# LinXueyuanStdio/LaTeX_OCR

Hardware: AMD Instinct MI355X
Metric: formula-images/sec training step (batch 64, 128x512) (higher is better)
Workload: dtype bf16

## Files before the change

latex_ocr_amd/csrc/conv_igemm.hip:

```cpp
#include "gemm.h"
#include "api_util.h"
#include "decoder_kernels.h"
#include "lxo_debug.h"
#include <stdlib.h>

namespace {

__device__ unsigned lxo_zero_line[8] = {0, 0, 0, 0, 0, 0, 0, 0};

constexpr int CBM = 256, CBN = 128, CBK = 64, CTH = 512;
constexpr int A_STAGE = CBM * CBK * 2, B_STAGE = CBN * CBK * 2, STAGE = A_STAGE + B_STAGE;

typedef __attribute__((address_space(1))) const void* gptr_t;
typedef __attribute__((address_space(3))) void* lptr_t;
LXO_DEV void glds16(const void* g, void* l) {
    __builtin_amdgcn_global_load_lds((gptr_t)(uintptr_t)g, (lptr_t)(uintptr_t)l, 16, 0, 0);
}

}

HIP_DYNAMIC_SHARED(char, lxo_conv_lds)

namespace {

constexpr int HTH = 4, HTW = 64, HPW = HTW + 2, HPH = HTH + 2, HPROWS = HPH * HPW;
constexpr int HPSLOTS = 7 * CTH;
constexpr int HPATCH = HPSLOTS * 16, HB_STAGE = CBN * CBK * 2;

#ifdef LXO_DIAG
#define LXO_DIAG_BIT(b) (p.diag & (b))
#else
#define LXO_DIAG_BIT(b) false
#endif
#define LXO_VMCNT(n) __builtin_amdgcn_s_waitcnt(0x0F70 | ((n) & 15) | (((n) >> 4) << 14))
#define LXO_LDS_BARRIER() do { __builtin_amdgcn_s_waitcnt(0xC07F); __builtin_amdgcn_s_barrier(); } while (0)

template <typename OT, int NJ>
__global__ __launch_bounds__(512) void conv_halo_kernel(GemmNT p, int tiles_n, int tiles_x, int tiles_y) {
    constexpr int BN = 64 * NJ, HBS = BN * CBK * 2;
    const int tid = threadIdx.x, lane = tid & 63, wave = tid >> 6;
    const int wm = wave >> 1, wn = wave & 1;
    const int nblk = gridDim.x, bid = blockIdx.x;
    const int q = nblk >> 3, r8 = nblk & 7, xcd = bid & 7, slot = bid >> 3;
    const int tile = (xcd < r8 ? xcd * (q + 1) : r8 * (q + 1) + (xcd - r8) * q) + slot;
    const int mt = tile / tiles_n, nt = tile - mt * tiles_n;
    const int tx_i = mt % tiles_x, ty_i = (mt / tiles_x) % tiles_y, b = mt / (tiles_x * tiles_y);
    const int oy0 = ty_i * HTH, ox0 = tx_i * HTW, n0 = nt * BN;
    const bf16_t* __restrict__ A = reinterpret_cast<const bf16_t*>(p.A);
    const bf16_t* __restrict__ Bp = reinterpret_cast<const bf16_t*>(p.Bp);
    const char* zline = reinterpret_cast<const char*>(lxo_zero_line);
    char* patch0 = lxo_conv_lds;
    char* bst0 = lxo_conv_lds + 2 * HPATCH;

    const int sch = tid & 7;
    long long a_off[7];
    int a_gch[7];
#pragma unroll
    for (int j = 0; j < 7; ++j) {
        const int prow = (tid >> 3) + 64 * j;
        const int py = prow / HPW, px = prow - py * HPW;
        const int iy = oy0 + py - p.pad, ix = ox0 + px - p.pad;
        const bool ok = prow < HPROWS && iy >= 0 && iy < p.H && ix >= 0 && ix < p.W;
        a_off[j] = ok ? (((long long)b * p.H + iy) * p.W + ix) * p.Cin : -1;
        a_gch[j] = (sch ^ ((prow >> 1) & 7)) << 3;
    }
    const int srow = tid >> 3;
    const bf16_t* b_ptr[NJ]; bool b_ok[NJ];
#pragma unroll
    for (int j = 0; j < NJ; ++j) {
        const int n = n0 + srow + 64 * j;
        b_ok[j] = n < p.N;
        b_ptr[j] = Bp + (long long)(b_ok[j] ? n : 0) * p.ldb + ((sch ^ ((srow >> 1) & 7)) << 3);
    }
    auto issue_patch = [&](int c, int buf) {
        char* dst = patch0 + buf * HPATCH;
#pragma unroll
        for (int j = 0; j < 7; ++j) {
            const void* src = a_off[j] >= 0 ? (const void*)(A + a_off[j] + c * CBK + a_gch[j]) : (const void*)zline;
            glds16(src, dst + (wave * 64 + 512 * j) * 16);
        }
    };
    auto issue_b = [&](int t, int stage) {
        const int c = t / 9, tap = t - 9 * c;
        const int k0 = tap * p.Cin + c * CBK;
        char* dst = bst0 + stage * HBS;
#pragma unroll
        for (int j = 0; j < NJ; ++j) {
            const void* src = b_ok[j] ? (const void*)(b_ptr[j] + k0) : (const void*)zline;
            glds16(src, dst + (wave * 64 + 512 * j) * 16);
        }
    };

    f32x16 acc[2][NJ];
#pragma unroll
    for (int i = 0; i < 2; ++i)
#pragma unroll
        for (int j = 0; j < NJ; ++j)
#pragma unroll
            for (int e = 0; e < 16; ++e) acc[i][j][e] = 0.f;

    int a_prow[2];
#pragma unroll
    for (int i = 0; i < 2; ++i) {
        const int rr = wm * 64 + i * 32 + (lane & 31);
        a_prow[i] = (rr >> 6) * HPW + (rr & 63);
    }
    int b_row[NJ];
#pragma unroll
    for (int j = 0; j < NJ; ++j) b_row[j] = wn * 32 * NJ + j * 32 + (lane & 31);

    const int nchunk = p.Cin / CBK, nk = nchunk * 9;
    issue_patch(0, 0);
    issue_b(0, 0);
    if (nk > 1) issue_b(1, 1);
    for (int t = 0; t < nk; ++t) {
        const int tm = t % 9;
        const bool patch_after = (tm == 5 || tm == 6) && (t / 9 + 1 < nchunk);
        const int nafter = ((t + 1 < nk) ? NJ : 0) + (patch_after ? 7 : 0);
        if (nafter == NJ + 7) LXO_VMCNT(NJ + 7);
        else if (nafter == 7) LXO_VMCNT(7);
        else if (nafter == NJ) LXO_VMCNT(NJ);
        else LXO_VMCNT(0);
        __builtin_amdgcn_s_barrier();
        if (t + 2 < nk) issue_b(t + 2, (t + 2) % 3);
        if (tm == 4 && t / 9 + 1 < nchunk) issue_patch(t / 9 + 1, (t / 9 + 1) & 1);
        const int c = t / 9, tap = t - 9 * c;
        const int kh = tap / 3, kw = tap - 3 * kh;
        const char* ps = patch0 + (c & 1) * HPATCH;
        const char* bs = bst0 + (t % 3) * HBS;
        const int shift = kh * HPW + kw;
#pragma unroll
        for (int ks = 0; ks < 4; ++ks) {
            const int kc = ks * 2 + (lane >> 5);
            u32x4 af[2], bfr[NJ];
#pragma unroll
            for (int i = 0; i < 2; ++i) {
                const int prow = a_prow[i] + shift;
                af[i] = *reinterpret_cast<const u32x4*>(ps + prow * 128 + ((kc ^ ((prow >> 1) & 7)) << 4));
            }
#pragma unroll
            for (int j = 0; j < NJ; ++j)
                bfr[j] = *reinterpret_cast<const u32x4*>(bs + b_row[j] * 128 + ((kc ^ ((b_row[j] >> 1) & 7)) << 4));
#pragma unroll
            for (int i = 0; i < 2; ++i)
#pragma unroll
                for (int j = 0; j < NJ; ++j)
                    acc[i][j] = __builtin_amdgcn_mfma_f32_32x32x16_bf16(__builtin_bit_cast(bf16x8_t, af[i]), __builtin_bit_cast(bf16x8_t, bfr[j]),
                                                                        acc[i][j], 0, 0, 0);
        }
    }

    OT* __restrict__ C = reinterpret_cast<OT*>(p.C);
    const bool plain = !p.out_pre && !p.addend && !p.relu_ref && !p.colsum && !p.accumulate && p.ldc == p.N && (p.N & 7) == 0;
    if (plain) {
        LXO_LDS_BARRIER();
        bf16_t* ot = reinterpret_cast<bf16_t*>(lxo_conv_lds);
        constexpr int OP = BN + 8;
#pragma unroll
        for (int j = 0; j < NJ; ++j) {
            const int nl = wn * 32 * NJ + j * 32 + (lane & 31);
            const int n = n0 + nl;
            const float bias = (p.bias && n < p.N) ? p.bias[n] : 0.f;
#pragma unroll
            for (int i = 0; i < 2; ++i)
#pragma unroll
                for (int e = 0; e < 16; ++e) {
                    const int ml = wm * 64 + i * 32 + (e & 3) + 8 * (e >> 2) + 4 * (lane >> 5);
                    float v = p.alpha * acc[i][j][e] + bias;
                    if (p.act == 1) v = fmaxf(v, 0.f);
                    else if (p.act == 2) v = tanhf(v);
                    ot[ml * OP + nl] = f2bf(v);
                }
        }
        LXO_LDS_BARRIER();
#pragma unroll
        for (int it = 0; it < 4 * NJ; ++it) {
            const int idx = tid + 512 * it, row = idx / (BN / 8), c8 = (idx % (BN / 8)) * 8;
            const int oy = oy0 + (row >> 6), ox = ox0 + (row & 63), n = n0 + c8;
            if (oy < p.Ho && ox < p.Wo && n < p.N)
                *reinterpret_cast<u32x4*>(C + (((long long)b * p.Ho + oy) * p.Wo + ox) * p.ldc + n) = *reinterpret_cast<const u32x4*>(ot + row * OP + c8);
        }
        return;
    }
    OT* __restrict__ Cpre = reinterpret_cast<OT*>(p.out_pre);
    const bf16_t* __restrict__ ref = reinterpret_cast<const bf16_t*>(p.relu_ref);
#pragma unroll
    for (int j = 0; j < NJ; ++j) {
        const int n = n0 + wn * 32 * NJ + j * 32 + (lane & 31);
        const bool n_ok = n < p.N;
        const float bias = (p.bias && n_ok) ? p.bias[n] : 0.f;
        float csum = 0.f;
#pragma unroll
        for (int i = 0; i < 2; ++i) {
#pragma unroll
            for (int e = 0; e < 16; ++e) {
                const int ml = wm * 64 + i * 32 + (e & 3) + 8 * (e >> 2) + 4 * (lane >> 5);
                const int oy = oy0 + (ml >> 6), ox = ox0 + (ml & 63);
                if (!(n_ok && oy < p.Ho && ox < p.Wo)) continue;
                const long long m = ((long long)b * p.Ho + oy) * p.Wo + ox;
                float v = p.alpha * acc[i][j][e] + bias;
                if (p.act == 1) v = fmaxf(v, 0.f);
                else if (p.act == 2) v = tanhf(v);
                const long long o = m * p.ldc + n;
                if (Cpre) Cpre[o] = from_f32<OT>(v);
                if (p.addend) v += p.addend[(m % p.addend_rows) * p.N + n];
                if (ref) v = (to_f32(ref[m * p.ldr + n]) > 0.f) ? v : 0.f;
                csum += v;
                if (p.accumulate) v += to_f32(C[o]);
                C[o] = from_f32<OT>(v);
            }
        }
        if (p.colsum) {
            csum += __shfl_xor(csum, 32);
            if (lane < 32 && n_ok) atomicAdd(&p.colsum[n], csum);
        }
    }
}

constexpr int QTH = 8, QTW = 32, QPW = QTW + 2, QPH = QTH + 2, QPROWS = QPH * QPW;

constexpr int WTHR = 256;
constexpr int WKC = 32;
constexpr int WPIX = 80;
constexpr int WPUNITS = QPROWS * 5;
constexpr int WPDMA = 7, WPATCHB = WPUNITS * 16;
constexpr int WWSTAGE = 32 * WKC * 2, WNST = 3;
constexpr int WLDS = 2 * WPATCHB + 4 * WNST * WWSTAGE;

template <int NJ, int EPI, int PH = 1, int PW = 1>
__global__ __launch_bounds__(256, 2) void conv_halo2wg_kernel(GemmNT p, int tiles_n, int tiles_x, int tiles_y) {
    constexpr int WBN = 32 * NJ;
    constexpr int NWM = 4 / NJ, RI = QTH / NWM;
    const int tid = threadIdx.x, lane = tid & 63;
    const int wave = __builtin_amdgcn_readfirstlane(tid >> 6);
    const int wn = wave % NJ, wm = wave / NJ;
    const int nblk = gridDim.x, bid = blockIdx.x;
    const int q = nblk >> 3, r8 = nblk & 7, xcd = bid & 7, slot = bid >> 3;
    const int tile = (xcd < r8 ? xcd * (q + 1) : r8 * (q + 1) + (xcd - r8) * q) + slot;
    const int mt = tile / tiles_n, nt = tile - mt * tiles_n;
    const int tx_i = mt % tiles_x, ty_i = (mt / tiles_x) % tiles_y, b = mt / (tiles_x * tiles_y);
    const int oy0 = ty_i * QTH, ox0 = tx_i * QTW, n0 = nt * WBN;
    const bf16_t* __restrict__ Bp = reinterpret_cast<const bf16_t*>(p.Bp);
    const unsigned wst_off = 2 * WPATCHB + wave * WNST * WWSTAGE;
    const unsigned m0base = __builtin_amdgcn_readfirstlane((unsigned)(uintptr_t)lxo_conv_lds);

    const lxo_rsrc_t rsA = lxo_make_rsrc(p.A, (unsigned)((long long)(p.M / (p.Ho * p.Wo)) * p.H * p.W * p.Cin * 2));
    const unsigned soffA = __builtin_amdgcn_readfirstlane((unsigned)(b * p.H * p.W * p.Cin * 2));
    unsigned a_src[WPDMA];
#pragma unroll
    for (int j = 0; j < WPDMA; ++j) {
        const int s = tid + WTHR * j;
        const int prow = s / 5, ch = s - 5 * prow;
        const int py = prow / QPW, px = prow - py * QPW;
        const int iy = oy0 + py - p.pad, ix = ox0 + px - p.pad;
        const bool ok = ch < 4 && prow < QPROWS && iy >= 0 && iy < p.H && ix >= 0 && ix < p.W;
        a_src[j] = ok ? (unsigned)(((iy * p.W + ix) * p.Cin + (ch << 3)) * 2) : LXO_BLDS_OOB;
    }
    unsigned w_src[2];
#pragma unroll
    for (int j = 0; j < 2; ++j) {
        const int r = 16 * j + (lane >> 2);
        w_src[j] = (unsigned)(((n0 + wn * 32 + r) * p.ldb + (((lane & 3) ^ ((r >> 2) & 3)) << 3)) * 2);
    }
    auto issue_patch_piece = [&](int c, int buf, int j) {
        if (LXO_DIAG_BIT(2)) c = 0;
        const unsigned so = soffA + (unsigned)(c * WKC * 2);
        if (j + 1 < WPDMA) LXO_BLDS16(a_src[j], rsA, so, lxo_conv_lds, m0base, buf * WPATCHB + wave * 1024 + 4096 * j);
        else if (wave * 64 + WTHR * j < WPUNITS) {
            if (tid + WTHR * j < WPUNITS) LXO_BLDS16(a_src[j], rsA, so, lxo_conv_lds, m0base, buf * WPATCHB + wave * 1024 + 4096 * j);
        }
    };
    auto issue_patch = [&](int c, int buf) {
#pragma unroll
        for (int j = 0; j < WPDMA; ++j) issue_patch_piece(c, buf, j);
    };
    auto issue_w = [&](int c, int tap, int stage) {
        const bf16_t* sb = LXO_DIAG_BIT(1) ? Bp : Bp + tap * p.Cin + c * WKC;
#pragma unroll
        for (int j = 0; j < 2; ++j) LXO_GLDS16_SADDR(w_src[j], sb, lxo_conv_lds, m0base, wst_off + stage * WWSTAGE + 1024 * j);
    };

    const int khalf = lane >> 5;

    const int a_lane0 = ((wm * RI) * QPW + (lane & 31)) * WPIX + khalf * 16;
    int w_lane[2];
#pragma unroll
    for (int ks = 0; ks < 2; ++ks)
        w_lane[ks] = (int)wst_off + (lane & 31) * 64 + (((2 * ks + khalf) ^ (((lane & 31) >> 2) & 3)) << 4);

    const int nchunk = p.Cin / WKC;
    const bool short_tile = __builtin_amdgcn_readfirstlane((RI == 8 && oy0 + 6 >= p.Ho) ? 1 : 0) != 0;
#define CSTAMP(i) do { if (p.dbg && tid == 0 && (i) < 64) p.dbg[(long long)bid * 64 + (i)] = __builtin_readcyclecounter(); } while (0)
    CSTAMP(0);
    if (p.dbg && tid == 0) p.dbg[(long long)bid * 64 + 63] = __builtin_amdgcn_s_getreg(63492);
    issue_patch(0, 0);
    issue_w(0, 0, 0);
    issue_w(0, 1, 1);
    issue_w(0, 2, 2);

    f32x16 acc[RI];
#pragma unroll
    for (int k = 0; k < 4; ++k) {
        const float* bsrc = p.bias ? p.bias + n0 + wn * 32 + 8 * k + 4 * khalf : reinterpret_cast<const float*>(lxo_zero_line);
        const f32x4 bq = *reinterpret_cast<const f32x4*>(bsrc);
#pragma unroll
        for (int i = 0; i < RI; ++i)
#pragma unroll
            for (int e = 0; e < 4; ++e) acc[i][4 * k + e] = bq[e];
    }


    u32x4 af[RI], bfr[2];
    int a_lane = a_lane0;
    auto fill = [&]() {
        bfr[0] = *reinterpret_cast<const u32x4*>(lxo_conv_lds + w_lane[0]);
#pragma unroll
        for (int i = 0; i < RI; ++i) af[i] = *reinterpret_cast<const u32x4*>(lxo_conv_lds + a_lane + i * QPW * WPIX);
    };

    LXO_VMCNT(0);
    __builtin_amdgcn_s_barrier();
    fill();
    for (int c = 0; c < nchunk; ++c) {
        const bool last = c + 1 == nchunk;
        CSTAMP(1 + c);
#pragma unroll
        for (int tap = 0; tap < 9; ++tap) {
            constexpr int NP = WPDMA;
            const int kh = tap / 3, kw = tap % 3;
            bfr[1] = *reinterpret_cast<const u32x4*>(lxo_conv_lds + w_lane[1] + (tap % 3) * WWSTAGE);
#pragma unroll
            for (int i = 0; i < RI; ++i) {
                if (RI == 8 && i >= 6 && short_tile) continue;
                acc[i] = __builtin_amdgcn_mfma_f32_32x32x16_bf16(__builtin_bit_cast(bf16x8_t, bfr[0]),
                                                                 __builtin_bit_cast(bf16x8_t, af[i]), acc[i], 0, 0, 0);
                af[i] = *reinterpret_cast<const u32x4*>(lxo_conv_lds + a_lane + ((i + kh) * QPW + kw) * WPIX + 32);
                __builtin_amdgcn_sched_barrier(0);
            }
            const int t3 = tap + 3 < 9 ? tap + 3 : tap + 3 - 9;
            const int kh1 = (tap + 1) / 3, kw1 = (tap + 1) % 3;
#pragma unroll
            for (int i = 0; i < RI; ++i) {
                if (RI == 8 && i >= 6 && short_tile) continue;
                acc[i] = __builtin_amdgcn_mfma_f32_32x32x16_bf16(__builtin_bit_cast(bf16x8_t, bfr[1]),
                                                                 __builtin_bit_cast(bf16x8_t, af[i]), acc[i], 0, 0, 0);
                if (i == 0 && (tap + 3 < 9 || !last)) issue_w(tap + 3 < 9 ? c : c + 1, t3, tap % 3);
                if (i == RI - 3) {
                    const int npa = ((tap - 2 >= 0 && tap - 2 < NP) ? 1 : 0) + ((tap - 1 >= 0 && tap - 1 < NP) ? 1 : 0);
                    const int npb = ((tap - 2 >= 0 && tap - 2 < NP - 1) ? 1 : 0) + ((tap - 1 >= 0 && tap - 1 < NP - 1) ? 1 : 0);
                    if (tap + 3 < 9 || !last) {
                        const int np = last ? 0 : (wave == 3 ? npb : npa);
                        if (np == 0) LXO_VMCNT(4); else if (np == 1) LXO_VMCNT(5); else LXO_VMCNT(6);
                    } else if (tap + 2 < 9) LXO_VMCNT(2);
                    else LXO_VMCNT(0);
                    if (tap + 1 < 9) bfr[0] = *reinterpret_cast<const u32x4*>(lxo_conv_lds + w_lane[0] + ((tap + 1) % 3) * WWSTAGE);
                    if (tap < NP && !last) issue_patch_piece(c + 1, (c + 1) & 1, tap);
                }
                if (tap + 1 < 9) af[i] = *reinterpret_cast<const u32x4*>(lxo_conv_lds + a_lane + ((i + kh1) * QPW + kw1) * WPIX);
                __builtin_amdgcn_sched_barrier(0);
            }
        }
        if (!last) {
            LXO_VMCNT(4);
            __builtin_amdgcn_s_barrier();
            a_lane = a_lane0 + ((c + 1) & 1) * WPATCHB;
            fill();
        }
    }
    const int nk = nchunk;

    CSTAMP(1 + nk);
    if constexpr (EPI == 0 || EPI == 2 || EPI == 4) {
        bf16_t* __restrict__ Cq = reinterpret_cast<bf16_t*>(p.C);
        constexpr int BP = WBN * 2 + 16;
        char* bt = lxo_conv_lds;
        const float floor_q = p.act == 1 ? 0.f : -3.0e38f;
        LXO_LDS_BARRIER();
        CSTAMP(40);
#pragma unroll
        for (int i = 0; i < RI; ++i)
#pragma unroll
            for (int k = 0; k < 4; ++k) {
                float v[4];
#pragma unroll
                for (int e = 0; e < 4; ++e) v[e] = fmaxf(acc[i][4 * k + e], floor_q);
                const u32x2 pk = {pack_bf2(v[0], v[1]), pack_bf2(v[2], v[3])};
                *reinterpret_cast<u32x2*>(bt + ((wm * RI + i) * 32 + (lane & 31)) * BP + (wn * 32 + 8 * k + 4 * khalf) * 2) = pk;
            }
        CSTAMP(41);
        LXO_LDS_BARRIER();
        CSTAMP(42);
        constexpr int CHQ = WBN / 8, RPQ = 256 / CHQ;
        const int cq = tid % CHQ;
        bf16_t* const tile0 = Cq + (((long long)b * p.Ho + oy0) * p.Wo + ox0) * p.ldc + n0 + cq * 8;
        if constexpr (EPI == 4) {
            constexpr int ph = PH, pw = PW;
            const int Hq = (p.Ho + ph - 1) / ph, Wq = (p.Wo + pw - 1) / pw;
            constexpr int tqw = QTW / pw, npool = (QTH / ph) * tqw;
            constexpr int NPP = npool * CHQ / 256;
            bf16_t* __restrict__ Pq = reinterpret_cast<bf16_t*>(p.pool_out);
            unsigned char* __restrict__ Mq = p.pool_mask;
#pragma unroll
            for (int it = 0; it < NPP; ++it) {
                const int pp = tid + 256 * it;
                const int pq = pp / CHQ, cqq = pp - pq * CHQ;
                const int pty = pq / tqw, ptx = pq - pty * tqw;
                const int oyq = oy0 / ph + pty, oxq = ox0 / pw + ptx;
                u32x4 w4[ph * pw];
#pragma unroll
                for (int q = 0; q < ph * pw; ++q)
                    w4[q] = *reinterpret_cast<const u32x4*>(bt + ((pty * ph + q / pw) * QTW + ptx * pw + q % pw) * BP + cqq * 16);
                float best[8]; int bq[8];
#pragma unroll
                for (int e = 0; e < 8; ++e) { best[e] = -3.0e38f; bq[e] = 0; }
#pragma unroll
                for (int q = 0; q < ph * pw; ++q) {
                    const bool ok = oy0 + pty * ph + q / pw < p.Ho && ox0 + ptx * pw + q % pw < p.Wo;
#pragma unroll
                    for (int e = 0; e < 8; ++e) {
                        const unsigned w = w4[q][e >> 1];
                        const float v = __uint_as_float((e & 1) ? (w & 0xffff0000u) : (w << 16));
                        const bool up = ok && v > best[e];
                        best[e] = up ? v : best[e]; bq[e] = up ? q : bq[e];
                    }
                }
                if (oyq < Hq && oxq < Wq) {
                    const long long o = (((long long)b * Hq + oyq) * Wq + oxq) * p.ldc + n0 + cqq * 8;
                    store8(Pq + o, best);
                    unsigned m0 = 0u, m1 = 0u;
#pragma unroll
                    for (int e = 0; e < 4; ++e) {
                        m0 |= (unsigned)(bq[e] | (best[e] > 0.f ? 4 : 0)) << (8 * e);
                        m1 |= (unsigned)(bq[4 + e] | (best[4 + e] > 0.f ? 4 : 0)) << (8 * e);
                    }
                    *reinterpret_cast<u32x2*>(Mq + o) = u32x2{m0, m1};
                }
            }
            if (!p.C) { CSTAMP(2 + nk); return; }
        }
        u32x4 q4[256 / RPQ];
#pragma unroll
        for (int it = 0; it < 256 / RPQ; ++it) q4[it] = *reinterpret_cast<const u32x4*>(bt + (tid / CHQ + RPQ * it) * BP + cq * 16);
        if constexpr (EPI == 2) {
            const bf16_t* const ref0 = reinterpret_cast<const bf16_t*>(p.relu_ref) + (((long long)b * p.Ho + oy0) * p.Wo + ox0) * p.ldr + n0 + cq * 8;
            u32x4 rf[256 / RPQ];
#pragma unroll
            for (int it = 0; it < 256 / RPQ; ++it) {
                const int row = tid / CHQ + RPQ * it, ty = row >> 5, tx = row & 31;
                const bool ok = oy0 + ty < p.Ho && ox0 + tx < p.Wo;
                rf[it] = *reinterpret_cast<const u32x4*>(ref0 + (ok ? (ty * p.Wo + tx) * p.ldr : 0));
            }
            float csum[8];
#pragma unroll
            for (int e = 0; e < 8; ++e) csum[e] = 0.f;
#pragma unroll
            for (int it = 0; it < 256 / RPQ; ++it) {
                const int row = tid / CHQ + RPQ * it, ty = row >> 5, tx = row & 31;
                const bool ok = oy0 + ty < p.Ho && ox0 + tx < p.Wo;
                u32x4 o;
#pragma unroll
                for (int d = 0; d < 4; ++d) {
                    const unsigned r = rf[it][d], v = q4[it][d];
                    const unsigned lo = (ok && (short)(r & 0xffffu) > 0) ? (v & 0xffffu) : 0u;
                    const unsigned hi = (ok && (int)r > 0 && (r >> 16) != 0u) ? (v & 0xffff0000u) : 0u;
                    o[d] = lo | hi;
                    csum[2 * d] += __uint_as_float(lo << 16);
                    csum[2 * d + 1] += __uint_as_float(hi);
                }
                if (ok) *reinterpret_cast<u32x4*>(tile0 + (ty * p.Wo + tx) * p.ldc) = o;
            }
            if (p.colsum || p.colsum_part) {
                float* cs = reinterpret_cast<float*>(lxo_conv_lds);
                LXO_LDS_BARRIER();
#pragma unroll
                for (int e = 0; e < 8; ++e) cs[(tid / CHQ) * WBN + cq * 8 + e] = csum[e];
                LXO_LDS_BARRIER();
                if (tid < WBN) {
                    float sres = 0.f;
#pragma unroll
                    for (int r = 0; r < RPQ; ++r) sres += cs[r * WBN + tid];
                    if (p.colsum_part) p.colsum_part[(long long)mt * p.N + n0 + tid] = sres;
                    else atomicAdd(&p.colsum[n0 + tid], sres);
                }
            }
            CSTAMP(2 + nk);
            return;
        }
#pragma unroll
        for (int it = 0; it < 256 / RPQ; ++it) {
            const int row = tid / CHQ + RPQ * it;
            const int ty = row >> 5, tx = row & 31;
            if (oy0 + ty < p.Ho && ox0 + tx < p.Wo && !LXO_DIAG_BIT(4)) *reinterpret_cast<u32x4*>(tile0 + (ty * p.Wo + tx) * p.ldc) = q4[it];
        }
        CSTAMP(2 + nk);
        return;
    }
    bf16_t* __restrict__ C = reinterpret_cast<bf16_t*>(p.C);
    bf16_t* __restrict__ Cpre = reinterpret_cast<bf16_t*>(p.out_pre);
    const bf16_t* __restrict__ ref = reinterpret_cast<const bf16_t*>(p.relu_ref);
    float* ot = reinterpret_cast<float*>(lxo_conv_lds);
    constexpr int OP = WBN + 4, CH = 4 * NJ, RPI = 256 / CH;
    const int c8 = (tid % CH) * 8, n = n0 + c8;
    float csum[8];
#pragma unroll
    for (int e = 0; e < 8; ++e) csum[e] = 0.f;
    const float act_floor = p.act == 1 ? 0.f : -3.0e38f;
    for (int pass = 0; pass < 4; ++pass) {
        LXO_LDS_BARRIER();
        CSTAMP(40 + 3 * pass);
#pragma unroll
        for (int pp = 0; pp < 4; ++pp) {
            if (pp == pass && wm == (2 * pp) / RI) {
#pragma unroll
                for (int ii = 0; ii < 2; ++ii)
#pragma unroll
                    for (int k = 0; k < 4; ++k) {
                        const int ib = (2 * pp) % RI;
                        const f32x4 q4 = {acc[ib + ii][4 * k], acc[ib + ii][4 * k + 1], acc[ib + ii][4 * k + 2], acc[ib + ii][4 * k + 3]};
                        *reinterpret_cast<f32x4*>(&ot[(ii * 32 + (lane & 31)) * OP + wn * 32 + 8 * k + 4 * khalf]) = q4;
                    }
            }
        }
        LXO_LDS_BARRIER();
        CSTAMP(41 + 3 * pass);
        constexpr int NIT = 64 / RPI;
        constexpr bool HAS_ADD = EPI == 1 || EPI == 3, HAS_REF = EPI == 2 || EPI == 3;
        f32x4 t0[NIT], t1[NIT], a0[NIT], a1[NIT], c0[NIT], c1[NIT];
        u32x4 rf[NIT];
        long long mrow[NIT];
        bool okr[NIT];
#pragma unroll
        for (int it = 0; it < NIT; ++it) {
            const int row = tid / CH + RPI * it;
            const int oy = oy0 + pass * 2 + (row >> 5), ox = ox0 + (row & 31);
            okr[it] = oy < p.Ho && ox < p.Wo;
            mrow[it] = okr[it] ? ((long long)b * p.Ho + oy) * p.Wo + ox : 0;
            t0[it] = *reinterpret_cast<const f32x4*>(ot + row * OP + c8); t1[it] = *reinterpret_cast<const f32x4*>(ot + row * OP + c8 + 4);
            if constexpr (HAS_ADD) {
                if (p.addend) {
                    const float* ad = p.addend + (mrow[it] % p.addend_rows) * p.N + n;
                    a0[it] = *reinterpret_cast<const f32x4*>(ad); a1[it] = *reinterpret_cast<const f32x4*>(ad + 4);
                } else { a0[it] = f32x4{0.f, 0.f, 0.f, 0.f}; a1[it] = a0[it]; }
            }
            if constexpr (HAS_REF) {
                if (ref) rf[it] = *reinterpret_cast<const u32x4*>(ref + mrow[it] * p.ldr + n);
                else rf[it] = u32x4{0x3f803f80u, 0x3f803f80u, 0x3f803f80u, 0x3f803f80u};
            }
            if constexpr (EPI == 3) {
                if (p.accumulate) {
                    float cv[8];
                    load8(C + mrow[it] * p.ldc + n, cv);
                    c0[it] = f32x4{cv[0], cv[1], cv[2], cv[3]}; c1[it] = f32x4{cv[4], cv[5], cv[6], cv[7]};
                } else { c0[it] = f32x4{0.f, 0.f, 0.f, 0.f}; c1[it] = c0[it]; }
            }
        }
#pragma unroll
        for (int it = 0; it < NIT; ++it) {
            float v[8];
#pragma unroll
            for (int e = 0; e < 8; ++e)
                v[e] = fmaxf(e < 4 ? t0[it][e] : t1[it][e - 4], act_floor);
            if constexpr (HAS_ADD) {
                if (Cpre && okr[it]) store8(Cpre + mrow[it] * p.ldc + n, v);
#pragma unroll
                for (int e = 0; e < 8; ++e) v[e] += (e < 4 ? a0[it][e] : a1[it][e - 4]);
            }
            if constexpr (HAS_REF) {
#pragma unroll
                for (int e = 0; e < 8; ++e) {
                    const unsigned w = rf[it][e >> 1];
                    const float rv = __uint_as_float((e & 1) ? (w & 0xffff0000u) : (w << 16));
                    v[e] = rv > 0.f ? v[e] : 0.f;
                }
            }
            if (okr[it]) {
#pragma unroll
                for (int e = 0; e < 8; ++e) csum[e] += v[e];
            }
            if constexpr (EPI == 3) {
#pragma unroll
                for (int e = 0; e < 8; ++e) v[e] += (e < 4 ? c0[it][e] : c1[it][e - 4]);
            }
            if (okr[it]) store8(C + mrow[it] * p.ldc + n, v);
        }
        CSTAMP(42 + 3 * pass);
    }
    CSTAMP(2 + nk);
    if (p.colsum || p.colsum_part) {
        LXO_LDS_BARRIER();
#pragma unroll
        for (int e = 0; e < 8; ++e) ot[(tid / CH) * OP + c8 + e] = csum[e];
        LXO_LDS_BARRIER();
        if (tid < WBN) {
            float sres = 0.f;
#pragma unroll
            for (int r = 0; r < RPI; ++r) sres += ot[r * OP + tid];
            if (p.colsum_part) p.colsum_part[(long long)mt * p.N + n0 + tid] = sres;
            else atomicAdd(&p.colsum[n0 + tid], sres);
        }
    }
}

}

static bool attr_needed(int family) {
    static bool done[4][64] = {};
    int dev = 0;
    if (hipGetDevice(&dev) != hipSuccess || dev < 0 || dev >= 64) return true;
    if (done[family][dev]) return false;
    done[family][dev] = true;
    return true;
}

static thread_local unsigned long long* g_conv_dbg = nullptr;
extern "C" int lxo_conv_debug(unsigned long long* buf) { g_conv_dbg = buf; return 0; }
int lxo_launch_conv_igemm(const GemmNT& p0, hipStream_t s) {
    GemmNT p = p0;
    p.dbg = g_conv_dbg;
#ifdef LXO_DIAG
    { static int diag = -1; if (diag < 0) { const char* e = getenv("LXO_CONV_DIAG"); diag = e ? atoi(e) : 0; } p.diag = diag; }
#else
    p.diag = 0;
#endif
    if (!p.conv || p.Cin % 64 || p.K % 64) return -2;
    static int use_2wg = -1;
    if (use_2wg < 0) { const char* e = getenv("LXO_CONV_2WG"); use_2wg = (e && e[0] == '0') ? 0 : 1; }
    const bool in_32bit = (long long)(p.M / (p.Ho * p.Wo)) * p.H * p.W * p.Cin * 2 < (1LL << 31);
    if (use_2wg && in_32bit && (p.N % 64) == 0 && p.act != 2 && p.alpha == 1.f) {
        constexpr int LDS4 = WLDS, LDS2 = WLDS;
        if (attr_needed(0)) {
            HIPRC(hipFuncSetAttribute(reinterpret_cast<const void*>(conv_halo2wg_kernel<4, 0>), hipFuncAttributeMaxDynamicSharedMemorySize, LDS4));
            HIPRC(hipFuncSetAttribute(reinterpret_cast<const void*>(conv_halo2wg_kernel<4, 1>), hipFuncAttributeMaxDynamicSharedMemorySize, LDS4));
            HIPRC(hipFuncSetAttribute(reinterpret_cast<const void*>(conv_halo2wg_kernel<4, 2>), hipFuncAttributeMaxDynamicSharedMemorySize, LDS4));
            HIPRC(hipFuncSetAttribute(reinterpret_cast<const void*>(conv_halo2wg_kernel<4, 3>), hipFuncAttributeMaxDynamicSharedMemorySize, LDS4));
            HIPRC(hipFuncSetAttribute(reinterpret_cast<const void*>(conv_halo2wg_kernel<4, 4, 2, 2>), hipFuncAttributeMaxDynamicSharedMemorySize, LDS4));
            HIPRC(hipFuncSetAttribute(reinterpret_cast<const void*>(conv_halo2wg_kernel<4, 4, 2, 1>), hipFuncAttributeMaxDynamicSharedMemorySize, LDS4));
            HIPRC(hipFuncSetAttribute(reinterpret_cast<const void*>(conv_halo2wg_kernel<4, 4, 1, 2>), hipFuncAttributeMaxDynamicSharedMemorySize, LDS4));
            HIPRC(hipFuncSetAttribute(reinterpret_cast<const void*>(conv_halo2wg_kernel<2, 0>), hipFuncAttributeMaxDynamicSharedMemorySize, LDS2));
            HIPRC(hipFuncSetAttribute(reinterpret_cast<const void*>(conv_halo2wg_kernel<2, 3>), hipFuncAttributeMaxDynamicSharedMemorySize, LDS2));
            HIPRC(hipFuncSetAttribute(reinterpret_cast<const void*>(conv_halo2wg_kernel<2, 1>), hipFuncAttributeMaxDynamicSharedMemorySize, LDS2));
            HIPRC(hipFuncSetAttribute(reinterpret_cast<const void*>(conv_halo2wg_kernel<2, 2>), hipFuncAttributeMaxDynamicSharedMemorySize, LDS2));
            HIPRC(hipFuncSetAttribute(reinterpret_cast<const void*>(conv_halo2wg_kernel<2, 4, 2, 2>), hipFuncAttributeMaxDynamicSharedMemorySize, LDS2));
            HIPRC(hipFuncSetAttribute(reinterpret_cast<const void*>(conv_halo2wg_kernel<2, 4, 2, 1>), hipFuncAttributeMaxDynamicSharedMemorySize, LDS2));
            HIPRC(hipFuncSetAttribute(reinterpret_cast<const void*>(conv_halo2wg_kernel<2, 4, 1, 2>), hipFuncAttributeMaxDynamicSharedMemorySize, LDS2));
        }
        const int B = p.M / (p.Ho * p.Wo);
        const int tiles_x = cdiv(p.Wo, QTW), tiles_y = cdiv(p.Ho, QTH);
        const bool has_add = p.addend || p.out_pre, has_ref = p.relu_ref || p.colsum || p.colsum_part;
        int epi = p.accumulate || (has_add && has_ref) ? 3 : (has_add ? 1 : (has_ref ? (p.relu_ref ? 2 : 3) : 0));
        if (p.pool_out) {
            if (epi != 0 || p.N % 128 || !p.pool_mask || p.pool_h < 1 || p.pool_h > 2 || p.pool_w < 1 || p.pool_w > 2 || p.pool_h * p.pool_w == 1) return -2;
            epi = 4;
        } else if (!p.C) return -2;
        const dim3 g4(B * tiles_x * tiles_y * (p.N / 128)), g2(B * tiles_x * tiles_y * (p.N / 64));
        if (p.colsum_part && (size_t)B * tiles_x * tiles_y * p.N > p.colsum_part_floats) return -6;
        static int small_thr = -1;
        if (small_thr < 0) { const char* e = getenv("LXO_CONV_SMALL"); small_thr = e ? atoi(e) : 256; }
        if (p.N % 128 == 0 && (int)g4.x >= small_thr) {
            if (epi == 0) hipLaunchKernelGGL((conv_halo2wg_kernel<4, 0>), g4, dim3(WTHR), LDS4, s, p, p.N / 128, tiles_x, tiles_y);
            else if (epi == 1) hipLaunchKernelGGL((conv_halo2wg_kernel<4, 1>), g4, dim3(WTHR), LDS4, s, p, p.N / 128, tiles_x, tiles_y);
            else if (epi == 2) hipLaunchKernelGGL((conv_halo2wg_kernel<4, 2>), g4, dim3(WTHR), LDS4, s, p, p.N / 128, tiles_x, tiles_y);
            else if (epi == 4 && p.pool_h == 2 && p.pool_w == 2) hipLaunchKernelGGL((conv_halo2wg_kernel<4, 4, 2, 2>), g4, dim3(WTHR), LDS4, s, p, p.N / 128, tiles_x, tiles_y);
            else if (epi == 4 && p.pool_h == 2) hipLaunchKernelGGL((conv_halo2wg_kernel<4, 4, 2, 1>), g4, dim3(WTHR), LDS4, s, p, p.N / 128, tiles_x, tiles_y);
            else if (epi == 4) hipLaunchKernelGGL((conv_halo2wg_kernel<4, 4, 1, 2>), g4, dim3(WTHR), LDS4, s, p, p.N / 128, tiles_x, tiles_y);
            else hipLaunchKernelGGL((conv_halo2wg_kernel<4, 3>), g4, dim3(WTHR), LDS4, s, p, p.N / 128, tiles_x, tiles_y);
        } else {
            if (epi == 0) hipLaunchKernelGGL((conv_halo2wg_kernel<2, 0>), g2, dim3(WTHR), LDS2, s, p, p.N / 64, tiles_x, tiles_y);
            else if (epi == 1) hipLaunchKernelGGL((conv_halo2wg_kernel<2, 1>), g2, dim3(WTHR), LDS2, s, p, p.N / 64, tiles_x, tiles_y);
            else if (epi == 2) hipLaunchKernelGGL((conv_halo2wg_kernel<2, 2>), g2, dim3(WTHR), LDS2, s, p, p.N / 64, tiles_x, tiles_y);
            else if (epi == 4 && p.pool_h == 2 && p.pool_w == 2) hipLaunchKernelGGL((conv_halo2wg_kernel<2, 4, 2, 2>), g2, dim3(WTHR), LDS2, s, p, p.N / 64, tiles_x, tiles_y);
            else if (epi == 4 && p.pool_h == 2) hipLaunchKernelGGL((conv_halo2wg_kernel<2, 4, 2, 1>), g2, dim3(WTHR), LDS2, s, p, p.N / 64, tiles_x, tiles_y);
            else if (epi == 4) hipLaunchKernelGGL((conv_halo2wg_kernel<2, 4, 1, 2>), g2, dim3(WTHR), LDS2, s, p, p.N / 64, tiles_x, tiles_y);
            else hipLaunchKernelGGL((conv_halo2wg_kernel<2, 3>), g2, dim3(WTHR), LDS2, s, p, p.N / 64, tiles_x, tiles_y);
        }
        if (p.colsum_part) return lxo_k_det_reduce(p.colsum_part, B * tiles_x * tiles_y, p.N, p.N, p.colsum, s);
        return (int)hipGetLastError();
    }
    if (p.pool_out || !p.C) return -2;
    if (p.colsum_part) return -7;
    {
        constexpr int LDSB = 2 * HPATCH + 3 * HB_STAGE, LDSB64 = 2 * HPATCH + 3 * (HB_STAGE / 2);
        if (attr_needed(2)) {
            HIPRC(hipFuncSetAttribute(reinterpret_cast<const void*>(conv_halo_kernel<bf16_t, 2>), hipFuncAttributeMaxDynamicSharedMemorySize, LDSB));
            HIPRC(hipFuncSetAttribute(reinterpret_cast<const void*>(conv_halo_kernel<bf16_t, 1>), hipFuncAttributeMaxDynamicSharedMemorySize, LDSB64));
        }
        const int B = p.M / (p.Ho * p.Wo);
        const int tiles_x = cdiv(p.Wo, HTW), tiles_y = cdiv(p.Ho, HTH);
        if (p.N <= 64) {
            const int tiles_n = cdiv(p.N, 64);
            hipLaunchKernelGGL((conv_halo_kernel<bf16_t, 1>), dim3(B * tiles_x * tiles_y * tiles_n), dim3(CTH), LDSB64, s, p, tiles_n, tiles_x, tiles_y);
            return (int)hipGetLastError();
        }
        const int tiles_n = cdiv(p.N, CBN);
        hipLaunchKernelGGL((conv_halo_kernel<bf16_t, 2>), dim3(B * tiles_x * tiles_y * tiles_n), dim3(CTH), LDSB, s, p, tiles_n, tiles_x, tiles_y);
        return (int)hipGetLastError();
    }
}
```

latex_ocr_amd/csrc/gemm.h:

```cpp
#pragma once
#include "lxo_common.h"

struct GemmNT {
    const void* A; const void* Bp; void* C;
    int M, N, K;
    int lda, ldb, ldc;
    int conv, H, W, Cin, Ho, Wo, pad;
    const float* bias;
    const float* addend; int addend_rows;
    int act;
    const void* relu_ref; int ldr;
    void* out_pre;
    int accumulate;
    float* colsum;
    float* colsum_part; size_t colsum_part_floats;
    float alpha;
    unsigned long long* dbg;
    void* pool_out; unsigned char* pool_mask; int pool_h, pool_w;
    int diag;
};

struct GemmTN {
    const void* A; const void* B; float* C;
    int M, I, J;
    int lda, ldb, ldc;
    int conv, H, W, Cin, Ho, Wo, pad;
    int nsplit, nbatch;
    long long strideA, strideB, strideC;
    int atomic;
    unsigned long long* dbg;
    float* det_slab; size_t det_floats;
};

int lxo_launch_gemm_nt(int dt, int a_f32, int c_f32, int small, const GemmNT& p, hipStream_t s);
int lxo_launch_gemm_tn(int dt, int a_f32, int b_f32, const GemmTN& p, hipStream_t s);

int lxo_launch_gemm_slab(int dt, const GemmNT& p, float* slab, long long slab_stride, hipStream_t s);

int lxo_launch_conv_igemm(const GemmNT& p, hipStream_t s);

int lxo_launch_gemm_nt_dma(const GemmNT& p, int c_f32, hipStream_t s);

int lxo_launch_gemm_tn_tr(const GemmTN& p, hipStream_t s);

int lxo_launch_conv_wgrad(const GemmTN& p, hipStream_t s);
```

latex_ocr_amd/csrc/model_encoder.hip:

```cpp
#include "impl.h"
#include "gemm.h"
#include "encoder_kernels.h"
#include "decoder_kernels.h"
#include "api_util.h"
#include "timing.h"

int lxo_impl_pack_weights(const Plan& P, const float* prm, void* wp, hipStream_t st) {
    const int dt = P.s.dtype, C = P.s.C, E = P.s.E, U = P.s.U, O = P.s.O, D = P.s.D, V = P.s.V;
    PackTable tab; memset(&tab, 0, sizeof(tab));
    int blocks = 0;
    auto add = [&](int kind, long long src, size_t dst, int K, int N, int lds, int ldd, int coff, int Kpad) {
        PackJob& j = tab.job[tab.n++];
        j.kind = kind; j.K = K; j.N = N; j.lds = lds; j.ldd = ldd; j.coff = coff; j.Kpad = Kpad; j.src = src; j.dst = (long long)dst;
        if (kind == 0) j.nblocks = cdiv(Kpad, 32) * cdiv(N, 32);
        else if (kind == 1) { long long t = cdivl((long long)K * Kpad, 256 * 4); j.nblocks = (int)(t < 1 ? 1 : (t > 512 ? 512 : t)); }
        else { long long t = cdivl((long long)K * 9 * N, 256 * 4); j.nblocks = (int)(t < 1 ? 1 : (t > 512 ? 512 : t)); }
        j.first_block = blocks; blocks += j.nblocks;
    };
    auto tr = [&](long long src, size_t dst, int K, int N, int ldd, int coff, int Kpad) { add(0, src, dst, K, N, N, ldd, coff, Kpad); };
    auto cp = [&](long long src, size_t dst, int R, int Ccols, int ldd, int Cpad) { add(1, src, dst, R, Ccols, Ccols, ldd, 0, Cpad); };
    for (int l = 1; l < 6; ++l) {
        const int ci = P.convCin[l], co = P.convCout[l];
        tr(P.poff[P.convW[l]], P.koff[K_CONV2_F + l - 1], 9 * ci, co, 9 * ci, 0, 9 * ci);
        add(2, P.poff[P.convW[l]], P.koff[K_CONV2_D + l - 1], ci, co, 0, 0, 0, 0);
    }
    if (P.cnn) {
        tr(P.poff[P_CONVS_W], P.koff[K_CONVS_F], 8 * C, C, 8 * C, 0, 8 * C);
        cp(P.poff[P_CONVS_W], P.koff[K_CONVS_D], 8 * C, C, C, C);
    }
    tr(P.poff[P_ATT_IMG], P.koff[K_ATT_IMG_T], C, E, C, 0, C);
    cp(P.poff[P_ATT_IMG], P.koff[K_ATT_IMG], C, E, E, E);
    {
        const int pid[3] = {P_WC0, P_WH0, P_WO0};
        const int nout[3] = {U, U, O};
        size_t offT = 0, offN = 0;
        for (int i = 0; i < 3; ++i) {
            tr(P.poff[pid[i]], P.koff[K_INIT_T] + offT, C, nout[i], C, 0, C);
            cp(P.poff[pid[i]], P.koff[K_INIT] + offN, C, nout[i], nout[i], nout[i]);
            offT += (size_t)nout[i] * C * P.esz; offN += (size_t)C * nout[i] * P.esz;
        }
    }
    const long long K = P.poff[P_LSTM_K];
    tr(K, P.koff[K_LSTM_XT], D, 4 * U, P.Dp, 0, P.Dp);
    tr(K + (long long)D * 4 * U, P.koff[K_LSTM_RT], P.XH, 4 * U, P.ldRT, 0, P.XH);
    cp(K, P.koff[K_LSTM], D + P.XH, 4 * U, P.ldK, 4 * U);
    tr(P.poff[P_ATT_H], P.koff[K_ATT_H_T], U, E, P.ldAHT, 0, U);
    cp(P.poff[P_ATT_H], P.koff[K_ATT_H], U, E, P.ldAH, E);
    tr(P.poff[P_OWH], P.koff[K_OW_T], U, O, P.ldOWT, 0, U);
    tr(P.poff[P_OWC], P.koff[K_OW_T], C, O, P.ldOWT, U, C);
    cp(P.poff[P_OWH], P.koff[K_OW], U, O, P.ldOW, O);
    cp(P.poff[P_OWC], P.koff[K_OW] + (size_t)U * P.ldOW * P.esz, C, O, P.ldOW, O);
    tr(P.poff[P_YWO], P.koff[K_YWO_T], O, V, O, 0, O);
    cp(P.poff[P_YWO], P.koff[K_YWO], O, V, P.Vp, P.Vp);
    if (P.rnn) {
        const int Ur = P.Ur;
        for (int d = 0; d < 2; ++d) {
            const long long k = P.poff[P_ROWF_K + 2 * d];
            tr(k, P.koff[K_ROWX_T + d], C, 4 * Ur, C, 0, C);
            cp(k, P.koff[K_ROWX + d], C, 4 * Ur, 4 * Ur, 4 * Ur);
            tr(k + (long long)C * 4 * Ur, P.koff[K_ROWH_T + d], Ur, 4 * Ur, Ur, 0, Ur);
            cp(k + (long long)C * 4 * Ur, P.koff[K_ROWH + d], Ur, 4 * Ur, 4 * Ur, 4 * Ur);
        }
    }
    return lxo_k_pack_batch(dt, tab, blocks, prm, wp, st);
}

static const char* conv_name(int Cin, int Cout, bool valid) {
    if (valid) return "conv6";
    if (Cin == 64) return "conv2";
    if (Cin == 128) return "conv3";
    return Cin == Cout ? "conv4" : "conv5";
}
static int conv_fwd(const Plan& P, const void* in, const void* wpk, const float* bias, void* out,
                    int H, int W, int Cin, int Cout, bool valid, const float* addend, int addend_rows,
                    void* out_pre, hipStream_t st) {
    GemmNT g; memset(&g, 0, sizeof(g));
    g.A = in; g.Bp = wpk; g.C = out;
    g.conv = 1; g.H = H; g.W = W; g.Cin = Cin;
    g.Ho = valid ? H - 2 : H; g.Wo = valid ? W - 2 : W; g.pad = valid ? 0 : 1;
    g.M = P.Be * g.Ho * g.Wo; g.N = Cout; g.K = 9 * Cin;
    g.lda = Cin; g.ldb = 9 * Cin; g.ldc = Cout;
    g.bias = bias; g.act = 1; g.alpha = 1.f;
    g.addend = addend; g.addend_rows = addend_rows > 0 ? addend_rows : 1; g.out_pre = out_pre;
    LxoTimed tm("conv_fwd", conv_name(Cin, Cout, valid), 2.0 * g.M * g.N * g.K, st);
    return lxo_launch_gemm_nt(P.s.dtype, 0, 0, 0, g, st);
}
static int conv_fwd_pool(const Plan& P, const void* in, const void* wpk, const float* bias, int H, int W, int Cin, int Cout,
                         void* pooled, void* mask, int ph, int pw, hipStream_t st) {
    GemmNT g; memset(&g, 0, sizeof(g));
    g.A = in; g.Bp = wpk; g.C = nullptr;
    g.conv = 1; g.H = H; g.W = W; g.Cin = Cin; g.Ho = H; g.Wo = W; g.pad = 1;
    g.M = P.Be * H * W; g.N = Cout; g.K = 9 * Cin;
    g.lda = Cin; g.ldb = 9 * Cin; g.ldc = Cout;
    g.bias = bias; g.act = 1; g.alpha = 1.f; g.addend_rows = 1;
    g.pool_out = pooled; g.pool_mask = (unsigned char*)mask; g.pool_h = ph; g.pool_w = pw;
    LxoTimed tm("conv_fwd", conv_name(Cin, Cout, false), 2.0 * g.M * g.N * g.K, st);
    return lxo_launch_gemm_nt(P.s.dtype, 0, 0, 0, g, st);
}
static int conv_dgrad(const Plan& P, const void* dout, const void* wd, void* din, int Hout, int Wout, int Cout,
                      int Hin, int Win, int Cin, bool valid, const void* relu_ref, float* colsum, DetScratch det, hipStream_t st) {
    GemmNT g; memset(&g, 0, sizeof(g));
    g.A = dout; g.Bp = wd; g.C = din;
    g.conv = 1; g.H = Hout; g.W = Wout; g.Cin = Cout;
    g.Ho = Hin; g.Wo = Win; g.pad = valid ? 2 : 1;
    g.M = P.Be * Hin * Win; g.N = Cin; g.K = 9 * Cout;
    g.lda = Cout; g.ldb = 9 * Cout; g.ldc = Cin;
    g.act = 0; g.alpha = 1.f; g.addend_rows = 1;
    g.relu_ref = relu_ref; g.ldr = Cin; g.colsum = colsum;
    if (P.det() && colsum) { g.colsum_part = det.p; g.colsum_part_floats = det.floats; }
    LxoTimed tm("conv_dgrad", conv_name(Cin, Cout, valid), 2.0 * P.Be * Hout * Wout * 9.0 * Cin * Cout, st);
    return lxo_launch_gemm_nt(P.s.dtype, 0, 0, 0, g, st);
}
static int conv_wgrad(const Plan& P, const void* in, const void* dout, float* dw, int H, int W, int Cin, int Cout,
                      bool valid, DetScratch det, hipStream_t st) {
    GemmTN g; memset(&g, 0, sizeof(g));
    g.A = in; g.B = dout; g.C = dw;
    g.conv = 1; g.H = H; g.W = W; g.Cin = Cin;
    g.Ho = valid ? H - 2 : H; g.Wo = valid ? W - 2 : W; g.pad = valid ? 0 : 1;
    g.M = P.Be * g.Ho * g.Wo; g.I = 9 * Cin; g.J = Cout;
    g.lda = Cin; g.ldb = Cout; g.ldc = Cout;
    const int tiles = cdiv(g.I, 128) * cdiv(g.J, 128);
    int ns = cdiv(1024, tiles);
    const int maxs = g.M / 256 > 0 ? g.M / 256 : 1;
    if (ns > maxs) ns = maxs;
    g.nsplit = ns < 1 ? 1 : ns; g.nbatch = 1; g.atomic = 1;
    if (P.bf && P.det()) { g.det_slab = det.p; g.det_floats = det.floats; }
    LxoTimed tm("conv_wgrad", conv_name(Cin, Cout, valid), 2.0 * g.M * g.I * g.J, st);
    return lxo_launch_gemm_tn(P.s.dtype, 0, 0, g, st);
}

int lxo_impl_encoder_fwd(const Plan& P, const float* prm, const void* wp, void* ws, const uint8_t* img, hipStream_t st) {
    const int dt = P.s.dtype, B = P.Be, C = P.s.C;
    void* p1 = P.ws<void>(ws, W_P1);
    RC(lxo_k_conv1_pool_fwd(dt, img, prm + P.poff[P_CONV1_W], prm + P.poff[P_CONV1_B], p1, B, P.s.H, P.s.W, st));
    const bool pf = P.pool_fused();
    if (pf) RC(conv_fwd_pool(P, p1, P.pk(wp, K_CONV2_F), prm + P.poff[P_CONV2_B], P.H1, P.W1, 64, 128, P.ws<void>(ws, W_P2), P.ws<void>(ws, W_M2), 2, 2, st));
    else {
    RC(conv_fwd(P, p1, P.pk(wp, K_CONV2_F), prm + P.poff[P_CONV2_B], P.ws<void>(ws, W_Y2), P.H1, P.W1, 64, 128, false, nullptr, 0, nullptr, st));
    RC(lxo_k_maxpool_fwd(dt, P.ws<void>(ws, W_Y2), P.ws<void>(ws, W_P2), B, P.H1, P.W1, 128, 2, 2, st));
    }
    RC(conv_fwd(P, P.ws<void>(ws, W_P2), P.pk(wp, K_CONV3_F), prm + P.poff[P_CONV3_B], P.ws<void>(ws, W_Y3), P.H2, P.W2, 128, 256, false, nullptr, 0, nullptr, st));
    if (!P.cnn && pf) {
        RC(conv_fwd_pool(P, P.ws<void>(ws, W_Y3), P.pk(wp, K_CONV4_F), prm + P.poff[P_CONV4_B], P.H2, P.W2, 256, 256, P.ws<void>(ws, W_P4), P.ws<void>(ws, W_M4), 2, 1, st));
        RC(conv_fwd_pool(P, P.ws<void>(ws, W_P4), P.pk(wp, K_CONV5_F), prm + P.poff[P_CONV5_B], P.H4, P.W2, 256, C, P.ws<void>(ws, W_P5), P.ws<void>(ws, W_M5), 1, 2, st));
    } else if (!P.cnn) {
        RC(conv_fwd(P, P.ws<void>(ws, W_Y3), P.pk(wp, K_CONV4_F), prm + P.poff[P_CONV4_B], P.ws<void>(ws, W_Y4), P.H2, P.W2, 256, 256, false, nullptr, 0, nullptr, st));
        RC(lxo_k_maxpool_fwd(dt, P.ws<void>(ws, W_Y4), P.ws<void>(ws, W_P4), B, P.H2, P.W2, 256, 2, 1, st));
        RC(conv_fwd(P, P.ws<void>(ws, W_P4), P.pk(wp, K_CONV5_F), prm + P.poff[P_CONV5_B], P.ws<void>(ws, W_Y5), P.H4, P.W2, 256, C, false, nullptr, 0, nullptr, st));
        RC(lxo_k_maxpool_fwd(dt, P.ws<void>(ws, W_Y5), P.ws<void>(ws, W_P5), B, P.H4, P.W2, C, 1, 2, st));
    } else {
        RC(conv_fwd(P, P.ws<void>(ws, W_Y3), P.pk(wp, K_CONV4_F), prm + P.poff[P_CONV4_B], P.ws<void>(ws, W_Y4), P.H2, P.W2, 256, 256, false, nullptr, 0, nullptr, st));
        RC(conv_fwd(P, P.ws<void>(ws, W_Y4), P.pk(wp, K_CONV5_F), prm + P.poff[P_CONV5_B], P.ws<void>(ws, W_Y5), P.H4, P.W2, 256, C, false, nullptr, 0, nullptr, st));
        RC(lxo_k_im2col_s2(dt, P.ws<void>(ws, W_Y5), P.ws<void>(ws, W_COLS), B, P.H4, P.W2, P.H6, P.W5, C, st));
        GemmNT g; memset(&g, 0, sizeof(g));
        g.A = P.ws<void>(ws, W_COLS); g.Bp = P.pk(wp, K_CONVS_F); g.C = P.ws<void>(ws, W_P5);
        g.M = B * P.H6 * P.W5; g.N = C; g.K = 8 * C; g.lda = 8 * C; g.ldb = 8 * C; g.ldc = C;
        g.bias = prm + P.poff[P_CONVS_B]; g.alpha = 1.f; g.addend_rows = 1;
        RC(lxo_launch_gemm_nt(dt, 0, 0, 0, g, st));
    }
    const bool pos = P.s.no_positional == 0;
    if (pos) RC(lxo_k_timing_signal(P.ws<float>(ws, W_POS), P.Hp, P.Wp, C, st));
    RC(conv_fwd(P, P.ws<void>(ws, W_P5), P.pk(wp, K_CONV6_F), prm + P.poff[P_CONV6_B], P.ws<void>(ws, W_IMG), P.H6, P.W5, C, C, true,
                pos ? P.ws<float>(ws, W_POS) : nullptr, P.R, P.ws<void>(ws, W_Y6), st));
    if (P.Be < P.s.B) {
        const size_t row = (size_t)P.R * C * P.esz;
        HIPRC(hipMemsetAsync((char*)P.ws<void>(ws, W_IMG) + (size_t)P.Be * row, 0, (size_t)(P.s.B - P.Be) * row, st));
        HIPRC(hipMemsetAsync((char*)P.ws<void>(ws, W_Y6) + (size_t)P.Be * row, 0, (size_t)(P.s.B - P.Be) * row, st));
    }
    if (P.rnn) RC(lxo_impl_rowenc_fwd(P, prm, wp, ws, st));
    return 0;
}

static thread_local hipStream_t g_enc_side = nullptr;
static thread_local hipEvent_t g_ev_x = nullptr, g_ev_free[3] = {nullptr, nullptr, nullptr}, g_ev_done = nullptr;
hipStream_t lxo_impl_encoder_side_stream() { return g_enc_side; }
int lxo_impl_set_encoder_side_stream(hipStream_t s) {
    g_enc_side = s;
    if (s && !g_ev_x) {
        HIPRC(hipEventCreateWithFlags(&g_ev_x, hipEventDisableTiming));
        HIPRC(hipEventCreateWithFlags(&g_ev_done, hipEventDisableTiming));
        for (int i = 0; i < 3; ++i) HIPRC(hipEventCreateWithFlags(&g_ev_free[i], hipEventDisableTiming));
    }
    return 0;
}

static const int XV[7] = {0, 0, 0, 1, 0, 2, 0}, YV[7] = {0, 0, 2, 2, 1, 1, 1};
static const int XC[7] = {0, 0, 1, 0, 1, 2, 0}, YC[7] = {0, 0, 2, 2, 0, 1, 1};

int lxo_impl_encoder_bwd(const Plan& P, const float* prm, const void* wp, void* ws, const uint8_t* img, float* grads,
                         int last_layer, int first_layer, hipStream_t st, void* const* ready) {
    const int dt = P.s.dtype, B = P.Be, C = P.s.C;
    void* const G[3] = {P.ws<void>(ws, W_G0), P.ws<void>(ws, W_G1), P.ws<void>(ws, W_G2)};
    const int* XB = P.cnn ? XC : XV; const int* YB = P.cnn ? YC : YV;
    auto gw = [&](int pid) { return grads + P.poff[pid]; };
    const DetScratch det = P.det_scratch(ws);
    auto dbp = [&](int pid) -> float* { return P.det() ? nullptr : gw(pid); };
    auto dbsum = [&](const void* x, long long rows, int Cc, int pid) -> int {
        if (!P.det()) return 0;
        return lxo_k_colsum_det(x, P.bf ? 1 : 0, Cc, gw(pid), rows, Cc, det, st);
    };
    hipStream_t side = ((P.det() && !P.bf) || lxo_timer_on()) ? nullptr : g_enc_side;
    const DetScratch det_w = side ? P.det_scratch_side(ws) : det;
    bool pending[3] = {false, false, false};
    auto acquire = [&](int i) -> int {
        if (side && pending[i]) { HIPRC(hipStreamWaitEvent(st, g_ev_free[i], 0)); pending[i] = false; }
        return 0;
    };
    auto wgrad = [&](const void* in, int xi, float* dw, int H, int W, int Cin, int Cout, bool valid, const void* dy_at = nullptr) -> int {
        const void* dy = dy_at ? dy_at : G[xi];
        if (!side) return conv_wgrad(P, in, dy, dw, H, W, Cin, Cout, valid, det, st);
        HIPRC(hipEventRecord(g_ev_x, st));
        HIPRC(hipStreamWaitEvent(side, g_ev_x, 0));
        RC(conv_wgrad(P, in, dy, dw, H, W, Cin, Cout, valid, det_w, side));
        HIPRC(hipEventRecord(g_ev_free[xi], side));
        pending[xi] = true;
        return 0;
    };
    if (P.rnn && last_layer >= 6) RC(lxo_impl_rowenc_bwd(P, prm, wp, ws, grads, st));
    for (int l = last_layer; l >= first_layer; --l) {
        void* const X = l >= 2 ? G[XB[l]] : nullptr;
        void* const Y = l >= 2 ? G[YB[l]] : nullptr;
        void* const Yup = l <= 5 ? G[YB[l + 1]] : nullptr;
        switch (l) {
        case 6:
            if (P.dimg_masked()) {
                const void* dy6 = P.ws<void>(ws, W_DIMG);
                RC(wgrad(P.ws<void>(ws, W_P5), XB[6], gw(P_CONV6_W), P.H6, P.W5, C, C, true, dy6));
                RC(acquire(YB[6]));
                RC(conv_dgrad(P, dy6, P.pk(wp, K_CONV6_D), Y, P.Hp, P.Wp, C, P.H6, P.W5, C, true, nullptr, nullptr, det, st));
                break;
            }
            RC(acquire(XB[6]));
            RC(lxo_k_mask_convert(dt, P.ws<float>(ws, W_DIMG), P.ws<void>(ws, W_Y6), X, dbp(P_CONV6_B), (long long)B * P.R, C, st));
            RC(dbsum(X, (long long)B * P.R, C, P_CONV6_B));
            RC(wgrad(P.ws<void>(ws, W_P5), XB[6], gw(P_CONV6_W), P.H6, P.W5, C, C, true));
            RC(acquire(YB[6]));
            RC(conv_dgrad(P, X, P.pk(wp, K_CONV6_D), Y, P.Hp, P.Wp, C, P.H6, P.W5, C, true, nullptr, nullptr, det, st));
            break;
        case 5:
            RC(acquire(XB[5]));
            if (P.cnn) {
                const int M = B * P.H6 * P.W5;
                if (P.det()) RC(dbsum(Yup, M, C, P_CONVS_B));
                else RC(lxo_k_colsum_ct(dt, Yup, gw(P_CONVS_B), M, C, st));
                GemmTN t; memset(&t, 0, sizeof(t));
                t.A = P.ws<void>(ws, W_COLS); t.B = Yup; t.C = gw(P_CONVS_W); t.M = M; t.I = 8 * C; t.J = C;
                t.lda = 8 * C; t.ldb = C; t.ldc = C;
                { int ns = M / 2048; if (ns < 1) ns = 1; if (ns > 16) ns = 16; t.nsplit = ns; }
                t.nbatch = 1; t.atomic = 1;
                if (P.bf && P.det()) { t.det_slab = det.p; t.det_floats = det.floats; }
                RC(lxo_launch_gemm_tn(dt, 0, 0, t, st));
                GemmNT g; memset(&g, 0, sizeof(g));
                g.A = Yup; g.Bp = P.pk(wp, K_CONVS_D); g.C = P.ws<void>(ws, W_COLS);
                g.M = M; g.N = 8 * C; g.K = C; g.lda = C; g.ldb = C; g.ldc = 8 * C; g.alpha = 1.f; g.addend_rows = 1;
                RC(lxo_launch_gemm_nt(dt, 0, 0, 0, g, st));
                RC(lxo_k_col2im_s2_relu(dt, P.ws<void>(ws, W_COLS), P.ws<void>(ws, W_Y5), X, dbp(P_CONV5_B), B, P.H4, P.W2, P.H6, P.W5, C, st));
                RC(dbsum(X, (long long)B * P.H4 * P.W2, C, P_CONV5_B));
                RC(wgrad(P.ws<void>(ws, W_Y4), XB[5], gw(P_CONV5_W), P.H4, P.W2, 256, C, false));
                RC(acquire(YB[5]));
                RC(conv_dgrad(P, X, P.pk(wp, K_CONV5_D), Y, P.H4, P.W2, C, P.H4, P.W2, 256, false, P.ws<void>(ws, W_Y4), gw(P_CONV4_B), det, st));
                break;
            }
            if (P.pool_fused()) RC(lxo_k_maxpool_mask_bwd(P.ws<unsigned char>(ws, W_M5), Yup, X, gw(P_CONV5_B), B, P.H4, P.W2, C, 1, 2, det, st));
            else RC(lxo_k_maxpool_relu_bwd(dt, P.ws<void>(ws, W_Y5), Yup, X, dbp(P_CONV5_B), B, P.H4, P.W2, C, 1, 2, st));
            if (!P.pool_fused()) RC(dbsum(X, (long long)B * P.H4 * P.W2, C, P_CONV5_B));
            RC(wgrad(P.ws<void>(ws, W_P4), XB[5], gw(P_CONV5_W), P.H4, P.W2, 256, C, false));
            RC(acquire(YB[5]));
            RC(conv_dgrad(P, X, P.pk(wp, K_CONV5_D), Y, P.H4, P.W2, C, P.H4, P.W2, 256, false, nullptr, nullptr, det, st));
            break;
        case 4:
            if (!P.cnn) {
                RC(acquire(XB[4]));
                if (P.pool_fused()) RC(lxo_k_maxpool_mask_bwd(P.ws<unsigned char>(ws, W_M4), Yup, X, gw(P_CONV4_B), B, P.H2, P.W2, 256, 2, 1, det, st));
                else RC(lxo_k_maxpool_relu_bwd(dt, P.ws<void>(ws, W_Y4), Yup, X, dbp(P_CONV4_B), B, P.H2, P.W2, 256, 2, 1, st));
                if (!P.pool_fused()) RC(dbsum(X, (long long)B * P.H2 * P.W2, 256, P_CONV4_B));
            }
            RC(wgrad(P.ws<void>(ws, W_Y3), XB[4], gw(P_CONV4_W), P.H2, P.W2, 256, 256, false));
            RC(acquire(YB[4]));
            RC(conv_dgrad(P, X, P.pk(wp, K_CONV4_D), Y, P.H2, P.W2, 256, P.H2, P.W2, 256, false, P.ws<void>(ws, W_Y3), gw(P_CONV3_B), det, st));
            break;
        case 3:
            RC(wgrad(P.ws<void>(ws, W_P2), XB[3], gw(P_CONV3_W), P.H2, P.W2, 128, 256, false));
            RC(acquire(YB[3]));
            RC(conv_dgrad(P, X, P.pk(wp, K_CONV3_D), Y, P.H2, P.W2, 256, P.H2, P.W2, 128, false, nullptr, nullptr, det, st));
            break;
        case 2:
            RC(acquire(XB[2]));
            if (P.pool_fused()) RC(lxo_k_maxpool_mask_bwd(P.ws<unsigned char>(ws, W_M2), Yup, X, gw(P_CONV2_B), B, P.H1, P.W1, 128, 2, 2, det, st));
            else RC(lxo_k_maxpool_relu_bwd(dt, P.ws<void>(ws, W_Y2), Yup, X, dbp(P_CONV2_B), B, P.H1, P.W1, 128, 2, 2, st));
            if (!P.pool_fused()) RC(dbsum(X, (long long)B * P.H1 * P.W1, 128, P_CONV2_B));
            RC(wgrad(P.ws<void>(ws, W_P1), XB[2], gw(P_CONV2_W), P.H1, P.W1, 64, 128, false));
            RC(acquire(YB[2]));
            RC(conv_dgrad(P, X, P.pk(wp, K_CONV2_D), Y, P.H1, P.W1, 128, P.H1, P.W1, 64, false, nullptr, nullptr, det, st));
            break;
        case 1:
            RC(lxo_k_conv1_pool_bwd(dt, img, prm + P.poff[P_CONV1_W], prm + P.poff[P_CONV1_B], G[YB[2]], gw(P_CONV1_W), gw(P_CONV1_B), B, P.s.H, P.s.W, det, st));
            break;
        default: return -4;
        }
        if (ready && ready[l]) {
            if (side) {
                HIPRC(hipEventRecord(g_ev_x, st));
                HIPRC(hipStreamWaitEvent(side, g_ev_x, 0));
                HIPRC(hipEventRecord((hipEvent_t)ready[l], side));
            } else HIPRC(hipEventRecord((hipEvent_t)ready[l], st));
        }
    }
    if (side) {
        HIPRC(hipEventRecord(g_ev_done, side));
        HIPRC(hipStreamWaitEvent(st, g_ev_done, 0));
    }
    return 0;
}
```

latex_ocr_amd/csrc/plan.h:

```cpp
#pragma once
#include "lxo.h"
#include "lxo_common.h"
#include "decoder_kernels.h"

enum ParamId {
    P_CONV1_W, P_CONV1_B, P_CONV2_W, P_CONV2_B, P_CONV3_W, P_CONV3_B, P_CONV4_W, P_CONV4_B,
    P_CONV5_W, P_CONV5_B,
    P_CONVS_W, P_CONVS_B,
    P_CONV6_W, P_CONV6_B,
    P_ROWF_K, P_ROWF_B, P_ROWB_K, P_ROWB_B,
    P_EMB, P_START, P_ATT_IMG, P_WC0, P_BC0, P_WH0, P_BH0, P_WO0, P_BO0,
    P_LSTM_K, P_LSTM_B, P_ATT_H, P_BETA, P_OWH, P_OWC, P_YWO, P_COUNT
};

enum PackId {
    K_CONV2_F, K_CONV3_F, K_CONV4_F, K_CONV5_F, K_CONV6_F,
    K_CONV2_D, K_CONV3_D, K_CONV4_D, K_CONV5_D, K_CONV6_D,
    K_ATT_IMG_T,
    K_ATT_IMG,
    K_INIT_T,
    K_INIT,
    K_LSTM_XT,
    K_LSTM_RT,
    K_LSTM,
    K_ATT_H_T,
    K_ATT_H,
    K_OW_T,
    K_OW,
    K_YWO_T,
    K_YWO,
    K_CONVS_F,
    K_CONVS_D,
    K_ROWX_T, K_ROWX_T1,
    K_ROWH_T, K_ROWH_T1,
    K_ROWH, K_ROWH1,
    K_ROWX, K_ROWX1,
    K_COUNT
};

enum WsId {
    W_P1, W_Y2, W_P2, W_Y3, W_Y4, W_P4, W_Y5, W_P5, W_Y6, W_IMG, W_POS,
    W_ATT_IMG, W_APART, W_MEAN, W_EMB_IN, W_ZX, W_REC, W_CS, W_GATES, W_ATTH, W_ALPHA, W_LOGITS,
    W_DLOGITS, W_LOSS, W_DOLOG, W_G, W_DHC, W_DE, W_DATTH, W_DZ, W_DXH, W_DCC, W_DIMG, W_DATTIMG,
    W_DEMB, W_DPRE0, W_DMEAN, W_G0, W_G1, W_G2, W_GNORM,
    W_S_K1, W_S_K2, W_S_K4, W_S_B1, W_S_B3, W_S_B4,
    W_RECB, W_GB, W_DZB, W_CARRYH, W_DEC_TX, W_DEC_TXE,
    W_DEC_IDS, W_DEC_FLAGS, W_DEC_EMB, W_DEC_ZX, W_DEC_LOGITS, W_BEAM_LP, W_BEAM_PAR, W_BEAM_TMP,
    W_COLS,
    W_RXT, W_RZX, W_RG, W_RC, W_RH, W_RHB, W_RDZ, W_RDZB, W_RDH, W_RDCC, W_RZERO,
    W_M2, W_M4, W_M5,
    W_ATT_EXP,
    W_XSYNC,
    W_DET,
    W_DATTHB,
    W_COUNT
};

struct Plan {
    lxo_shape s;
    bool bf;
    size_t esz;
    int H1, W1, H2, W2, H4, W5, H6, Hp, Wp, R;
    bool cnn;
    bool rnn;
    int Be;
    int Ur;
    int convCin[6], convCout[6], convW[6], convB[6];
    int Vp, Dp, Rp, XH, HC, REC;
    int OFF_HT, OFF_CTX;
    int ldRT, ldAHT, ldOWT, ldOW, ldAH, ldK;
    int RECB, GBP, DZBP;
    Drop drop(int t, int row0) const;
    long long poff[P_COUNT], pcount[P_COUNT], ptotal;
    size_t koff[K_COUNT], ktotal;
    size_t woff[W_COUNT], wbytes[W_COUNT], wtotal;

    explicit Plan(const lxo_shape& sh, int beam = 1);
    int validate(char* msg, size_t n) const;
    int attn_chunks(int nv) const;

    bool pool_fused() const;
    bool dimg_masked() const { return bf && s.E % 32 == 0 && !rnn; }
    bool det() const { return !bf || s.deterministic != 0; }
    bool att_exp() const;
    DetScratch det_scratch(void* base) const { DetScratch d = {nullptr, 0}; if (det()) { d.p = ws<float>(base, W_DET); d.floats = wbytes[W_DET] / 4 / (bf ? 2 : 1); } return d; }
    DetScratch det_scratch_side(void* base) const { DetScratch d = {nullptr, 0}; if (det() && bf) { d.floats = wbytes[W_DET] / 8; d.p = ws<float>(base, W_DET) + d.floats; } return d; }
    template <class T> T* ws(void* base, WsId id) const { return reinterpret_cast<T*>(static_cast<char*>(base) + woff[id]); }
    const void* pk(const void* base, PackId id) const { return static_cast<const char*>(base) + koff[id]; }
    void* pk(void* base, PackId id) const { return static_cast<char*>(base) + koff[id]; }
};

const char* lxo_param_name(int id);
const char* lxo_param_name_mode(int id, int encoder_cnn);
```

latex_ocr_amd/csrc/plan.hip:

```cpp
#include "plan.h"
#include <stdio.h>
#include <string.h>
#include <stdlib.h>

static const char* kParamNames[P_COUNT] = {
    "Encoder/convolutional_encoder/conv2d/kernel", "Encoder/convolutional_encoder/conv2d/bias",
    "Encoder/convolutional_encoder/conv2d_1/kernel", "Encoder/convolutional_encoder/conv2d_1/bias",
    "Encoder/convolutional_encoder/conv2d_2/kernel", "Encoder/convolutional_encoder/conv2d_2/bias",
    "Encoder/convolutional_encoder/conv2d_3/kernel", "Encoder/convolutional_encoder/conv2d_3/bias",
    "Encoder/convolutional_encoder/conv2d_4/kernel", "Encoder/convolutional_encoder/conv2d_4/bias",
    "Encoder/convolutional_encoder/conv2d_strided/kernel", "Encoder/convolutional_encoder/conv2d_strided/bias",
    "Encoder/convolutional_encoder/conv2d_5/kernel", "Encoder/convolutional_encoder/conv2d_5/bias",
    "Encoder/row_encoder/bidirectional_rnn/fw/lstm_cell/kernel", "Encoder/row_encoder/bidirectional_rnn/fw/lstm_cell/bias",
    "Encoder/row_encoder/bidirectional_rnn/bw/lstm_cell/kernel", "Encoder/row_encoder/bidirectional_rnn/bw/lstm_cell/bias",
    "Decoder/embedding_table", "Decoder/start_token",
    "Decoder/AttentionCell/att_img/kernel",
    "Decoder/AttentionCell/att_mechanism/W_c_0", "Decoder/AttentionCell/att_mechanism/b_c_0",
    "Decoder/AttentionCell/att_mechanism/W_h_0", "Decoder/AttentionCell/att_mechanism/b_h_0",
    "Decoder/AttentionCell/att_mechanism/W_o_0", "Decoder/AttentionCell/att_mechanism/b_o_0",
    "Decoder/AttentionCell/rnn/lstm_cell/kernel", "Decoder/AttentionCell/rnn/lstm_cell/bias",
    "Decoder/AttentionCell/rnn/att_mechanism/dense/kernel", "Decoder/AttentionCell/rnn/att_mechanism/att_beta",
    "Decoder/AttentionCell/rnn/o_W_h", "Decoder/AttentionCell/rnn/o_W_c", "Decoder/AttentionCell/rnn/y_W_o",
};
const char* lxo_param_name(int id) { return (id >= 0 && id < P_COUNT) ? kParamNames[id] : ""; }
const char* lxo_param_name_mode(int id, int encoder_cnn) {
    if (encoder_cnn) {
        switch (id) {
        case P_CONVS_W: return "Encoder/convolutional_encoder/conv2d_5/kernel";
        case P_CONVS_B: return "Encoder/convolutional_encoder/conv2d_5/bias";
        case P_CONV6_W: return "Encoder/convolutional_encoder/conv2d_6/kernel";
        case P_CONV6_B: return "Encoder/convolutional_encoder/conv2d_6/bias";
        default: break;
        }
    }
    return lxo_param_name(id);
}

static const char* kWsNames[W_COUNT] = {
    "p1", "y2", "p2", "y3", "y4", "p4", "y5", "p5", "y6", "img", "pos",
    "att_img", "att_part", "mean", "emb_in", "zx", "rec", "cs", "gates", "att_h", "alpha", "logits",
    "dlogits", "loss", "do_log", "g", "dhc", "de", "datth", "dz", "dxh", "dcc", "d_img", "d_att_img",
    "d_emb", "dpre0", "dmean", "g0", "g1", "g2", "gnorm",
    "s_k1", "s_k2", "s_k4", "s_b1", "s_b3", "s_b4",
    "recb", "gb", "dzb", "carry_h", "dec_tx", "dec_txe",
    "dec_ids", "dec_flags", "dec_emb", "dec_zx", "dec_logits", "beam_lp", "beam_par", "beam_tmp",
    "cols",
    "rxt", "rzx", "rg", "rc", "rh", "rhb", "rdz", "rdzb", "rdh", "rdcc", "rzero",
    "m2", "m4", "m5",
    "att_exp", "xdec_sync", "det_part", "datth_b",
};
const char* lxo_ws_name(int id) { return (id >= 0 && id < W_COUNT) ? kWsNames[id] : ""; }

static inline int cd2(int n) { return (n + 1) / 2; }
static inline size_t al256(size_t n) { return (n + 255) / 256 * 256; }

Plan::Plan(const lxo_shape& sh, int ) : s(sh) {
    bf = s.dtype == LXO_BF16;
    esz = bf ? 2 : 4;
    const int B = s.B, C = s.C, E = s.E, U = s.U, O = s.O, D = s.D, V = s.V, T = s.T > 0 ? s.T : 1;
    H1 = cd2(s.H); W1 = cd2(s.W);
    H2 = cd2(H1); W2 = cd2(W1);
    cnn = s.encoder_cnn != 0;
    rnn = s.encoder_rnn != 0;
    Be = (s.live_B > 0 && s.live_B < s.B && !rnn) ? s.live_B : s.B;
    Ur = C / 2;
    H4 = cnn ? H2 : cd2(H2);
    W5 = cd2(W2);
    H6 = cnn ? cd2(H2) : H4;
    Hp = H6 - 2; Wp = W5 - 2;
    R = Hp > 0 && Wp > 0 ? Hp * Wp : 0;
    const int ci[6] = {1, 64, 128, 256, 256, C}, co[6] = {64, 128, 256, 256, C, C};
    const int wid[6] = {P_CONV1_W, P_CONV2_W, P_CONV3_W, P_CONV4_W, P_CONV5_W, P_CONV6_W};
    for (int i = 0; i < 6; ++i) { convCin[i] = ci[i]; convCout[i] = co[i]; convW[i] = wid[i]; convB[i] = wid[i] + 1; }
    Vp = (V + 31) / 32 * 32;
    Dp = (D + 63) / 64 * 64;
    Rp = (R + 7) / 8 * 8;
    XH = O + U; HC = U + C; OFF_HT = O + U; OFF_CTX = O + 2 * U; REC = O + 2 * U + C;
    const int WPAD = 128;
    ldRT = XH + WPAD; ldAHT = U + WPAD; ldOWT = HC + WPAD; ldOW = O + WPAD; ldAH = E + WPAD; ldK = 4 * U + WPAD;
    RECB = REC + WPAD; GBP = O + WPAD; DZBP = 4 * U + WPAD;

    long long cnt[P_COUNT];
    for (int i = 0; i < 6; ++i) { cnt[convW[i]] = 9LL * ci[i] * co[i]; cnt[convB[i]] = co[i]; }
    cnt[P_CONVS_W] = cnn ? 8LL * C * C : 0; cnt[P_CONVS_B] = cnn ? C : 0;
    cnt[P_ROWF_K] = cnt[P_ROWB_K] = rnn ? (long long)(C + Ur) * 4 * Ur : 0; cnt[P_ROWF_B] = cnt[P_ROWB_B] = rnn ? 4LL * Ur : 0;
    cnt[P_EMB] = (long long)V * D; cnt[P_START] = D; cnt[P_ATT_IMG] = (long long)C * E;
    cnt[P_WC0] = (long long)C * U; cnt[P_BC0] = U; cnt[P_WH0] = (long long)C * U; cnt[P_BH0] = U;
    cnt[P_WO0] = (long long)C * O; cnt[P_BO0] = O;
    cnt[P_LSTM_K] = (long long)(D + O + U) * 4 * U; cnt[P_LSTM_B] = 4LL * U;
    cnt[P_ATT_H] = (long long)U * E; cnt[P_BETA] = E;
    cnt[P_OWH] = (long long)U * O; cnt[P_OWC] = (long long)C * O; cnt[P_YWO] = (long long)O * V;
    ptotal = 0;
    for (int i = 0; i < P_COUNT; ++i) { poff[i] = ptotal; pcount[i] = cnt[i]; ptotal += cnt[i]; }

    size_t kb[K_COUNT];
    for (int l = 1; l < 6; ++l) {
        kb[K_CONV2_F + l - 1] = (size_t)co[l] * 9 * ci[l] * esz;
        kb[K_CONV2_D + l - 1] = (size_t)ci[l] * 9 * co[l] * esz;
    }
    kb[K_ATT_IMG_T] = (size_t)E * C * esz; kb[K_ATT_IMG] = (size_t)C * E * esz;
    kb[K_INIT_T] = (size_t)(2 * U + O) * C * esz; kb[K_INIT] = (size_t)C * (2 * U + O) * esz;
    kb[K_LSTM_XT] = (size_t)4 * U * Dp * esz; kb[K_LSTM_RT] = (size_t)4 * U * ldRT * esz;
    kb[K_LSTM] = (size_t)(D + O + U) * ldK * esz;
    kb[K_ATT_H_T] = (size_t)E * ldAHT * esz; kb[K_ATT_H] = (size_t)U * ldAH * esz;
    kb[K_OW_T] = (size_t)O * ldOWT * esz; kb[K_OW] = (size_t)HC * ldOW * esz;
    kb[K_YWO_T] = (size_t)V * O * esz; kb[K_YWO] = (size_t)O * Vp * esz;
    kb[K_CONVS_F] = cnn ? (size_t)8 * C * C * esz : 0; kb[K_CONVS_D] = kb[K_CONVS_F];
    for (int d = 0; d < 2; ++d) {
        kb[K_ROWX_T + d] = rnn ? (size_t)4 * Ur * C * esz : 0; kb[K_ROWX + d] = kb[K_ROWX_T + d];
        kb[K_ROWH_T + d] = rnn ? (size_t)4 * Ur * Ur * esz : 0; kb[K_ROWH + d] = kb[K_ROWH_T + d];
    }
    ktotal = 0;
    for (int i = 0; i < K_COUNT; ++i) { koff[i] = ktotal; ktotal += al256(kb[i] + 64); }

    const size_t f4 = 4;
    size_t wb[W_COUNT];
    memset(wb, 0, sizeof(wb));
    const size_t BL = (size_t)B;
    wb[W_P1] = BL * H1 * W1 * 64 * esz;
    wb[W_Y2] = BL * H1 * W1 * 128 * esz;  wb[W_P2] = BL * H2 * W2 * 128 * esz;
    wb[W_Y3] = BL * H2 * W2 * 256 * esz;  wb[W_Y4] = BL * H2 * W2 * 256 * esz;
    wb[W_P4] = cnn ? 0 : BL * H4 * W2 * 256 * esz;
    wb[W_Y5] = BL * H4 * W2 * C * esz;    wb[W_P5] = BL * H6 * W5 * C * esz;
    wb[W_COLS] = cnn ? BL * H6 * W5 * 8 * C * esz : 0;
    wb[W_Y6] = BL * R * C * esz;          wb[W_IMG] = BL * R * C * esz;
    wb[W_POS] = (size_t)R * C * f4;
    if (rnn) {
        const size_t TM = (size_t)B * (Hp > 0 ? Hp : 0) * (Wp > 0 ? Wp : 0), Mr = (size_t)B * (Hp > 0 ? Hp : 0);
        wb[W_RXT] = TM * C * esz;
        wb[W_RZX] = 2 * TM * 4 * Ur * f4;
        wb[W_RG] = 2 * TM * 4 * Ur * f4; wb[W_RC] = 2 * TM * Ur * f4; wb[W_RH] = 2 * TM * Ur * f4;
        wb[W_RHB] = bf ? 2 * TM * Ur * 2 : 0;
        wb[W_RDZ] = 2 * TM * 4 * Ur * f4; wb[W_RDZB] = bf ? 2 * TM * 4 * Ur * 2 : 0;
        wb[W_RDH] = TM * C * f4; wb[W_RDCC] = 2 * Mr * Ur * f4; wb[W_RZERO] = Mr * 4 * Ur * f4;
    }
    wb[W_M2] = bf ? BL * H2 * W2 * 128 : 0;
    wb[W_M4] = (bf && !cnn) ? BL * H4 * W2 * 256 : 0;
    wb[W_M5] = (bf && !cnn) ? BL * H6 * W5 * C : 0;
    wb[W_ATT_EXP] = bf ? BL * R * E * esz : 0;
    wb[W_XSYNC] = bf ? 2 * ((size_t)4096 + (384u << 10)) : 8192;
    wb[W_DET] = 8192;
    if (!bf || s.deterministic) {
        size_t need = BL * (size_t)((R + 15) / 16) * E * f4;
        const size_t floor_ = (size_t)1024 * (4 * U > 2048 ? 4 * U : 2048) * f4;
        wb[W_DET] = need > floor_ ? need : floor_;
        const size_t wg = (size_t)264 * 9 * 64 * 128 * f4;
        if (bf && wb[W_DET] < wg) wb[W_DET] = wg;
        if (bf) wb[W_DET] = 2 * ((wb[W_DET] + 255) / 256 * 256);
    }
    const int nb = s.beam > 1 ? s.beam : 1;
    const size_t BK_ = BL * nb;
    const size_t TB = (size_t)T * B;
    wb[W_DATTHB] = bf ? TB * E * 2 : 0;
    wb[W_ATT_IMG] = BL * R * E * esz;
    wb[W_APART] = BK_ * 32 * (C + 16) * f4;
    wb[W_MEAN] = BL * C * f4;
    wb[W_EMB_IN] = TB * Dp * esz;
    wb[W_ZX] = TB * 4 * U * f4;
    wb[W_REC] = (size_t)(T + 1) * B * REC * f4;
    wb[W_CS] = (size_t)(T + 1) * B * U * f4;
    wb[W_GATES] = TB * 4 * U * f4;
    wb[W_ATTH] = TB * E * f4;
    wb[W_ALPHA] = TB * Rp * f4;
    wb[W_LOGITS] = TB * Vp * f4;
    wb[W_DLOGITS] = TB * Vp * esz;
    wb[W_LOSS] = 64;
    wb[W_DOLOG] = TB * O * f4;
    wb[W_G] = TB * O * f4;
    wb[W_DHC] = TB * HC * f4;
    wb[W_DE] = TB * Rp * f4;
    wb[W_DATTH] = TB * E * f4;
    wb[W_DZ] = TB * 4 * U * f4;
    wb[W_DXH] = BL * XH * f4;
    wb[W_DCC] = BL * U * f4;
    wb[W_DIMG] = BL * R * C * f4;
    wb[W_DATTIMG] = BL * R * E * esz;
    wb[W_DEMB] = TB * D * f4;
    wb[W_DPRE0] = BL * (2 * U + O) * f4;
    wb[W_DMEAN] = BL * C * f4;
    size_t gmax = wb[W_Y2];
    const size_t cand[] = {wb[W_P1], wb[W_P2], wb[W_Y3], wb[W_Y4], wb[W_P4], wb[W_Y5], wb[W_P5], wb[W_Y6]};
    for (size_t c : cand) if (c > gmax) gmax = c;
    wb[W_G0] = gmax; wb[W_G1] = gmax; wb[W_G2] = gmax;
    wb[W_GNORM] = 64;
    wb[W_S_K1] = (size_t)(XH / 128) * BK_ * 4 * U * f4;
    wb[W_S_K2] = (size_t)(U / 128) * BK_ * E * f4;
    wb[W_S_K4] = (size_t)(HC / 128) * BK_ * O * f4;
    wb[W_S_B1] = (size_t)(O / 128) * BL * HC * f4;
    wb[W_S_B3] = (size_t)(E / 128) * BL * U * f4;
    wb[W_S_B4] = (size_t)(4 * U / 128) * BL * XH * f4;
    wb[W_RECB] = bf ? (size_t)(T + 1) * B * RECB * 2 : 0;
    wb[W_GB] = bf ? TB * GBP * 2 : 0;
    wb[W_DZB] = bf ? TB * DZBP * 2 : 0;
    wb[W_CARRYH] = BL * U * f4;
    const int ms = s.max_steps > 0 ? s.max_steps : 0;
    if (ms > 0) {
        wb[W_DEC_IDS] = BK_ * ms * 4 + 64;
        wb[W_DEC_FLAGS] = 256 + BK_ * 4;
        wb[W_DEC_EMB] = BK_ * Dp * esz;
        wb[W_DEC_TX] = (size_t)(V + 1) * 4 * U * f4;
        wb[W_DEC_TXE] = (size_t)(V + 1) * Dp * esz;
        wb[W_DEC_ZX] = BK_ * 4 * U * f4;
        wb[W_DEC_LOGITS] = BK_ * Vp * f4;
        wb[W_BEAM_LP] = BK_ * 2 * f4;
        wb[W_BEAM_PAR] = BK_ * ms * 4;
        wb[W_BEAM_TMP] = 3 * (BK_ * REC + BK_ * U) * f4 / 3 + BK_ * 64;
        if (wb[W_BEAM_TMP] < BK_ * Vp * f4) wb[W_BEAM_TMP] = BK_ * Vp * f4;
        const size_t recd = 2 * BK_ * REC * f4, csd = 2 * BK_ * U * f4;
        if (wb[W_REC] < recd) wb[W_REC] = recd;
        if (bf && wb[W_RECB] < 2 * BK_ * RECB * 2) wb[W_RECB] = 2 * BK_ * RECB * 2;
        if (wb[W_CS] < csd) wb[W_CS] = csd;
        if (wb[W_GATES] < BK_ * 4 * U * f4) wb[W_GATES] = BK_ * 4 * U * f4;
        if (wb[W_ATTH] < BK_ * E * f4) wb[W_ATTH] = BK_ * E * f4;
        if (wb[W_ALPHA] < BK_ * Rp * f4) wb[W_ALPHA] = BK_ * Rp * f4;
        if (wb[W_ZX] < BK_ * 4 * U * f4) wb[W_ZX] = BK_ * 4 * U * f4;
    }
    wtotal = 0;
    for (int i = 0; i < W_COUNT; ++i) { wbytes[i] = wb[i]; woff[i] = wtotal; wtotal += al256(wb[i] + 256); }
}

int Plan::attn_chunks(int nv) const {
    static int target = -1;
    if (target < 0) { const char* e = getenv("LXO_ATT_WGS"); target = (e && atoi(e) > 0) ? atoi(e) : 512; }
    int nch = (target + nv - 1) / nv;
    if (nch > 16) nch = 16;
    const int by_rows = R / 32 > 0 ? R / 32 : 1;
    if (nch > by_rows) nch = by_rows;
    const int need = (R + 1023) / 1024;
    if (nch < need) nch = need;
    return nch < 1 ? 1 : nch;
}

int Plan::validate(char* msg, size_t n) const {
#define BAD(cond, text) if (cond) { snprintf(msg, n, "lxo_shape invalid: %s", text); return -10; }
    BAD(s.B <= 0 || s.H <= 0 || s.W <= 0, "B/H/W must be positive");
    BAD(Hp <= 0 || Wp <= 0, "image too small: need ceil(H/8) >= 3 and ceil(W/8) >= 3");
    BAD(s.V < 4, "V < 4");
    BAD(s.C != 512 && s.C != 256 && s.C != 128, "C must be 128/256/512");
    BAD(s.E % 128 || s.U % 128 || s.O % 128 || s.E <= 0 || s.U <= 0 || s.O <= 0, "E, U, O must be positive multiples of 128");
    BAD(s.D % 8 || s.D <= 0, "D must be a positive multiple of 8");
    BAD(s.dtype != LXO_F32 && s.dtype != LXO_BF16, "dtype");
    BAD(s.E > 1024 || s.C > 512, "E <= 1024, C <= 512");
    BAD(R > 16384, "more than 16384 regions");
    BAD(s.encoder_rnn && s.C != 512 && s.C != 256, "encoder_rnn needs C in {256, 512} (C/2 units per direction, multiples of 128)");
#undef BAD
    return 0;
}

bool Plan::att_exp() const {
    static int v = -1;
    if (v < 0) { const char* e = getenv("LXO_ATT_EXP"); v = (e && atoi(e) == 0) ? 0 : 1; }
    return bf && v == 1 && s.E <= 256 && (long long)s.B * R * s.E % 8 == 0;
}
bool Plan::pool_fused() const {
    static int v = -1;
    if (v < 0) { const char* e = getenv("LXO_POOL_FUSED"); v = (e && atoi(e) == 0) ? 0 : 1; }
    static int halo = -1;
    if (halo < 0) { const char* b2 = getenv("LXO_CONV_2WG"); halo = (b2 && b2[0] == '0') ? 0 : 1; }
    return bf && v == 1 && halo == 1 && s.C % 128 == 0;
}
Drop Plan::drop(int t, int row0) const {
    Drop d = {0u, 1.f, (unsigned)s.dropout_seed, t, row0, s.B};
    if (s.keep_prob > 0.f && s.keep_prob < 1.f) {
        d.thr = (unsigned)(s.keep_prob * 16777216.0f);
        if (d.thr == 0u) d.thr = 1u;
        d.inv_keep = 1.f / s.keep_prob;
    }
    return d;
}
```

Measured before the change: 8667.

## Fuse max-unpool backward into conv dgrad epilogue with rotating gradient buffers

After: 8718 (median of 6 runs). No clear change (+0.6%).

```diff
diff --git a/latex_ocr_amd/csrc/conv_igemm.hip b/latex_ocr_amd/csrc/conv_igemm.hip
--- a/latex_ocr_amd/csrc/conv_igemm.hip
+++ b/latex_ocr_amd/csrc/conv_igemm.hip
@@ -370,7 +370,7 @@
     const int nk = nchunk;
 
     CSTAMP(1 + nk);
-    if constexpr (EPI == 0 || EPI == 2 || EPI == 4) {
+    if constexpr (EPI == 0 || EPI == 2 || EPI == 4 || EPI == 5) {
         bf16_t* __restrict__ Cq = reinterpret_cast<bf16_t*>(p.C);
         constexpr int BP = WBN * 2 + 16;
         char* bt = lxo_conv_lds;
@@ -441,6 +441,22 @@
         u32x4 q4[256 / RPQ];
 #pragma unroll
         for (int it = 0; it < 256 / RPQ; ++it) q4[it] = *reinterpret_cast<const u32x4*>(bt + (tid / CHQ + RPQ * it) * BP + cq * 16);
+        auto colsum_out = [&](const float (&csum)[8]) {
+            if (p.colsum || p.colsum_part) {
+                float* cs = reinterpret_cast<float*>(lxo_conv_lds);
+                LXO_LDS_BARRIER();
+#pragma unroll
+                for (int e = 0; e < 8; ++e) cs[(tid / CHQ) * WBN + cq * 8 + e] = csum[e];
+                LXO_LDS_BARRIER();
+                if (tid < WBN) {
+                    float sres = 0.f;
+#pragma unroll
+                    for (int r = 0; r < RPQ; ++r) sres += cs[r * WBN + tid];
+                    if (p.colsum_part) p.colsum_part[(long long)mt * p.N + n0 + tid] = sres;
+                    else atomicAdd(&p.colsum[n0 + tid], sres);
+                }
+            }
+        };
         if constexpr (EPI == 2) {
             const bf16_t* const ref0 = reinterpret_cast<const bf16_t*>(p.relu_ref) + (((long long)b * p.Ho + oy0) * p.Wo + ox0) * p.ldr + n0 + cq * 8;
             u32x4 rf[256 / RPQ];
@@ -469,20 +485,55 @@
                 }
                 if (ok) *reinterpret_cast<u32x4*>(tile0 + (ty * p.Wo + tx) * p.ldc) = o;
             }
-            if (p.colsum || p.colsum_part) {
-                float* cs = reinterpret_cast<float*>(lxo_conv_lds);
-                LXO_LDS_BARRIER();
-#pragma unroll
-                for (int e = 0; e < 8; ++e) cs[(tid / CHQ) * WBN + cq * 8 + e] = csum[e];
-                LXO_LDS_BARRIER();
-                if (tid < WBN) {
-                    float sres = 0.f;
-#pragma unroll
-                    for (int r = 0; r < RPQ; ++r) sres += cs[r * WBN + tid];
-                    if (p.colsum_part) p.colsum_part[(long long)mt * p.N + n0 + tid] = sres;
-                    else atomicAdd(&p.colsum[n0 + tid], sres);
+            colsum_out(csum);
+            CSTAMP(2 + nk);
+            return;
+        }
+        if constexpr (EPI == 5) {
+            constexpr int ph = PH, pw = PW;
+            const int Hf = p.pool_H, Wf = p.pool_W;
+            const unsigned char* const mk0 = p.pool_mask + (((long long)b * p.Ho + oy0) * p.Wo + ox0) * p.ldc + n0 + cq * 8;
+            bf16_t* const dy0 = reinterpret_cast<bf16_t*>(p.pool_out) + (((long long)b * Hf + oy0 * ph) * Wf + ox0 * pw) * p.ldc + n0 + cq * 8;
+            u32x2 mk[256 / RPQ];
+#pragma unroll
+            for (int it = 0; it < 256 / RPQ; ++it) {
+                const int row = tid / CHQ + RPQ * it, ty = row >> 5, tx = row & 31;
+                const bool ok = oy0 + ty < p.Ho && ox0 + tx < p.Wo;
+                mk[it] = *reinterpret_cast<const u32x2*>(mk0 + (ok ? (ty * p.Wo + tx) * p.ldc : 0));
+            }
+            float csum[8];
+#pragma unroll
+            for (int e = 0; e < 8; ++e) csum[e] = 0.f;
+#pragma unroll
+            for (int it = 0; it < 256 / RPQ; ++it) {
+                const int row = tid / CHQ + RPQ * it, ty = row >> 5, tx = row & 31;
+                const bool ok = oy0 + ty < p.Ho && ox0 + tx < p.Wo;
+                const u32x4 g4 = q4[it]; const u32x2 m2 = mk[it];
+                unsigned gm[4];
+#pragma unroll
+                for (int d = 0; d < 4; ++d) {
+                    const unsigned mlo = (m2[d >> 1] >> (16 * (d & 1))) & 0xffu, mhi = (m2[d >> 1] >> (16 * (d & 1) + 8)) & 0xffu;
+                    const unsigned lo = (ok && (mlo & 4u)) ? (g4[d] & 0xffffu) : 0u, hi = (ok && (mhi & 4u)) ? (g4[d] & 0xffff0000u) : 0u;
+                    gm[d] = lo | hi;
+                    csum[2 * d] += __uint_as_float(lo << 16); csum[2 * d + 1] += __uint_as_float(hi);
                 }
-            }
+                if (Cq && ok) *reinterpret_cast<u32x4*>(tile0 + (ty * p.Wo + tx) * p.ldc) = g4;
+#pragma unroll
+                for (int qy = 0; qy < ph; ++qy)
+#pragma unroll
+                    for (int qx = 0; qx < pw; ++qx) {
+                        const unsigned q = (unsigned)(qy * pw + qx);
+                        u32x4 o;
+#pragma unroll
+                        for (int d = 0; d < 4; ++d) {
+                            const unsigned mlo = (m2[d >> 1] >> (16 * (d & 1))) & 3u, mhi = (m2[d >> 1] >> (16 * (d & 1) + 8)) & 3u;
+                            o[d] = (mlo == q ? (gm[d] & 0xffffu) : 0u) | (mhi == q ? (gm[d] & 0xffff0000u) : 0u);
+                        }
+                        if (ok && (oy0 + ty) * ph + qy < Hf && (ox0 + tx) * pw + qx < Wf)
+                            *reinterpret_cast<u32x4*>(dy0 + ((ty * ph + qy) * Wf + tx * pw + qx) * p.ldc) = o;
+                    }
+            }
+            colsum_out(csum);
             CSTAMP(2 + nk);
             return;
         }
@@ -612,6 +663,24 @@
     return true;
 }
 
+static bool conv_use_2wg() {
+    static int use_2wg = -1;
+    if (use_2wg < 0) { const char* e = getenv("LXO_CONV_2WG"); use_2wg = (e && e[0] == '0') ? 0 : 1; }
+    return use_2wg != 0;
+}
+static bool conv_in_32bit(const GemmNT& p) { return (long long)(p.M / (p.Ho * p.Wo)) * p.H * p.W * p.Cin * 2 < (1LL << 31); }
+static bool conv_takes_2wg(const GemmNT& p) { return conv_use_2wg() && conv_in_32bit(p) && (p.N % 64) == 0 && p.act != 2 && p.alpha == 1.f; }
+int lxo_conv_igemm_route_refusal(const GemmNT& p) {
+    if (!p.pool_route || !p.conv || p.Cin % 64 || p.K % 64 || p.Ho <= 0 || p.Wo <= 0) return -2;
+    if (!conv_takes_2wg(p)) return -2;
+    if (p.addend || p.out_pre || p.relu_ref || p.accumulate || p.bias || p.act != 0 || p.ldc != p.N) return -2;
+    if (!p.pool_out || !p.pool_mask || p.pool_h < 1 || p.pool_h > 2 || p.pool_w < 1 || p.pool_w > 2 || p.pool_h * p.pool_w == 1) return -2;
+    if (p.Ho != cdiv(p.pool_H, p.pool_h) || p.Wo != cdiv(p.pool_W, p.pool_w)) return -2;
+    const long long B = p.M / (p.Ho * p.Wo);
+    if (B * p.pool_H * p.pool_W * p.N * 2 >= (1LL << 31)) return -2;
+    if (p.colsum_part && (size_t)B * cdiv(p.Wo, QTW) * cdiv(p.Ho, QTH) * p.N > p.colsum_part_floats) return -6;
+    return 0;
+}
 static thread_local unsigned long long* g_conv_dbg = nullptr;
 extern "C" int lxo_conv_debug(unsigned long long* buf) { g_conv_dbg = buf; return 0; }
 int lxo_launch_conv_igemm(const GemmNT& p0, hipStream_t s) {
@@ -622,11 +691,9 @@
 #else
     p.diag = 0;
 #endif
+    if (p.pool_route) { if (const int rc = lxo_conv_igemm_route_refusal(p)) return rc; }
     if (!p.conv || p.Cin % 64 || p.K % 64) return -2;
-    static int use_2wg = -1;
-    if (use_2wg < 0) { const char* e = getenv("LXO_CONV_2WG"); use_2wg = (e && e[0] == '0') ? 0 : 1; }
-    const bool in_32bit = (long long)(p.M / (p.Ho * p.Wo)) * p.H * p.W * p.Cin * 2 < (1LL << 31);
-    if (use_2wg && in_32bit && (p.N % 64) == 0 && p.act != 2 && p.alpha == 1.f) {
+    if (conv_takes_2wg(p)) {
         constexpr int LDS4 = WLDS, LDS2 = WLDS;
         if (attr_needed(0)) {
             HIPRC(hipFuncSetAttribute(reinterpret_cast<const void*>(conv_halo2wg_kernel<4, 0>), hipFuncAttributeMaxDynamicSharedMemorySize, LDS4));
@@ -643,12 +710,19 @@
             HIPRC(hipFuncSetAttribute(reinterpret_cast<const void*>(conv_halo2wg_kernel<2, 4, 2, 2>), hipFuncAttributeMaxDynamicSharedMemorySize, LDS2));
             HIPRC(hipFuncSetAttribute(reinterpret_cast<const void*>(conv_halo2wg_kernel<2, 4, 2, 1>), hipFuncAttributeMaxDynamicSharedMemorySize, LDS2));
             HIPRC(hipFuncSetAttribute(reinterpret_cast<const void*>(conv_halo2wg_kernel<2, 4, 1, 2>), hipFuncAttributeMaxDynamicSharedMemorySize, LDS2));
+            HIPRC(hipFuncSetAttribute(reinterpret_cast<const void*>(conv_halo2wg_kernel<4, 5, 2, 2>), hipFuncAttributeMaxDynamicSharedMemorySize, LDS4));
+            HIPRC(hipFuncSetAttribute(reinterpret_cast<const void*>(conv_halo2wg_kernel<4, 5, 2, 1>), hipFuncAttributeMaxDynamicSharedMemorySize, LDS4));
+            HIPRC(hipFuncSetAttribute(reinterpret_cast<const void*>(conv_halo2wg_kernel<4, 5, 1, 2>), hipFuncAttributeMaxDynamicSharedMemorySize, LDS4));
+            HIPRC(hipFuncSetAttribute(reinterpret_cast<const void*>(conv_halo2wg_kernel<2, 5, 2, 2>), hipFuncAttributeMaxDynamicSharedMemorySize, LDS2));
+            HIPRC(hipFuncSetAttribute(reinterpret_cast<const void*>(conv_halo2wg_kernel<2, 5, 2, 1>), hipFuncAttributeMaxDynamicSharedMemorySize, LDS2));
+            HIPRC(hipFuncSetAttribute(reinterpret_cast<const void*>(conv_halo2wg_kernel<2, 5, 1, 2>), hipFuncAttributeMaxDynamicSharedMemorySize, LDS2));
         }
         const int B = p.M / (p.Ho * p.Wo);
         const int tiles_x = cdiv(p.Wo, QTW), tiles_y = cdiv(p.Ho, QTH);
         const bool has_add = p.addend || p.out_pre, has_ref = p.relu_ref || p.colsum || p.colsum_part;
         int epi = p.accumulate || (has_add && has_ref) ? 3 : (has_add ? 1 : (has_ref ? (p.relu_ref ? 2 : 3) : 0));
-        if (p.pool_out) {
+        if (p.pool_route) epi = 5;
+        else if (p.pool_out) {
             if (epi != 0 || p.N % 128 || !p.pool_mask || p.pool_h < 1 || p.pool_h > 2 || p.pool_w < 1 || p.pool_w > 2 || p.pool_h * p.pool_w == 1) return -2;
             epi = 4;
         } else if (!p.C) return -2;
@@ -663,6 +737,9 @@
             else if (epi == 4 && p.pool_h == 2 && p.pool_w == 2) hipLaunchKernelGGL((conv_halo2wg_kernel<4, 4, 2, 2>), g4, dim3(WTHR), LDS4, s, p, p.N / 128, tiles_x, tiles_y);
             else if (epi == 4 && p.pool_h == 2) hipLaunchKernelGGL((conv_halo2wg_kernel<4, 4, 2, 1>), g4, dim3(WTHR), LDS4, s, p, p.N / 128, tiles_x, tiles_y);
             else if (epi == 4) hipLaunchKernelGGL((conv_halo2wg_kernel<4, 4, 1, 2>), g4, dim3(WTHR), LDS4, s, p, p.N / 128, tiles_x, tiles_y);
+            else if (epi == 5 && p.pool_h == 2 && p.pool_w == 2) hipLaunchKernelGGL((conv_halo2wg_kernel<4, 5, 2, 2>), g4, dim3(WTHR), LDS4, s, p, p.N / 128, tiles_x, tiles_y);
+            else if (epi == 5 && p.pool_h == 2) hipLaunchKernelGGL((conv_halo2wg_kernel<4, 5, 2, 1>), g4, dim3(WTHR), LDS4, s, p, p.N / 128, tiles_x, tiles_y);
+            else if (epi == 5) hipLaunchKernelGGL((conv_halo2wg_kernel<4, 5, 1, 2>), g4, dim3(WTHR), LDS4, s, p, p.N / 128, tiles_x, tiles_y);
             else hipLaunchKernelGGL((conv_halo2wg_kernel<4, 3>), g4, dim3(WTHR), LDS4, s, p, p.N / 128, tiles_x, tiles_y);
         } else {
             if (epi == 0) hipLaunchKernelGGL((conv_halo2wg_kernel<2, 0>), g2, dim3(WTHR), LDS2, s, p, p.N / 64, tiles_x, tiles_y);
@@ -671,6 +748,9 @@
             else if (epi == 4 && p.pool_h == 2 && p.pool_w == 2) hipLaunchKernelGGL((conv_halo2wg_kernel<2, 4, 2, 2>), g2, dim3(WTHR), LDS2, s, p, p.N / 64, tiles_x, tiles_y);
             else if (epi == 4 && p.pool_h == 2) hipLaunchKernelGGL((conv_halo2wg_kernel<2, 4, 2, 1>), g2, dim3(WTHR), LDS2, s, p, p.N / 64, tiles_x, tiles_y);
             else if (epi == 4) hipLaunchKernelGGL((conv_halo2wg_kernel<2, 4, 1, 2>), g2, dim3(WTHR), LDS2, s, p, p.N / 64, tiles_x, tiles_y);
+            else if (epi == 5 && p.pool_h == 2 && p.pool_w == 2) hipLaunchKernelGGL((conv_halo2wg_kernel<2, 5, 2, 2>), g2, dim3(WTHR), LDS2, s, p, p.N / 64, tiles_x, tiles_y);
+            else if (epi == 5 && p.pool_h == 2) hipLaunchKernelGGL((conv_halo2wg_kernel<2, 5, 2, 1>), g2, dim3(WTHR), LDS2, s, p, p.N / 64, tiles_x, tiles_y);
+            else if (epi == 5) hipLaunchKernelGGL((conv_halo2wg_kernel<2, 5, 1, 2>), g2, dim3(WTHR), LDS2, s, p, p.N / 64, tiles_x, tiles_y);
             else hipLaunchKernelGGL((conv_halo2wg_kernel<2, 3>), g2, dim3(WTHR), LDS2, s, p, p.N / 64, tiles_x, tiles_y);
         }
         if (p.colsum_part) return lxo_k_det_reduce(p.colsum_part, B * tiles_x * tiles_y, p.N, p.N, p.colsum, s);
diff --git a/latex_ocr_amd/csrc/gemm.h b/latex_ocr_amd/csrc/gemm.h
--- a/latex_ocr_amd/csrc/gemm.h
+++ b/latex_ocr_amd/csrc/gemm.h
@@ -17,6 +17,7 @@
     float alpha;
     unsigned long long* dbg;
     void* pool_out; unsigned char* pool_mask; int pool_h, pool_w;
+    int pool_route, pool_H, pool_W;
     int diag;
 };
 
@@ -38,6 +39,7 @@
 int lxo_launch_gemm_slab(int dt, const GemmNT& p, float* slab, long long slab_stride, hipStream_t s);
 
 int lxo_launch_conv_igemm(const GemmNT& p, hipStream_t s);
+int lxo_conv_igemm_route_refusal(const GemmNT& p);
 
 int lxo_launch_gemm_nt_dma(const GemmNT& p, int c_f32, hipStream_t s);
 
diff --git a/latex_ocr_amd/csrc/model_encoder.hip b/latex_ocr_amd/csrc/model_encoder.hip
--- a/latex_ocr_amd/csrc/model_encoder.hip
+++ b/latex_ocr_amd/csrc/model_encoder.hip
@@ -97,8 +97,9 @@
     LxoTimed tm("conv_fwd", conv_name(Cin, Cout, false), 2.0 * g.M * g.N * g.K, st);
     return lxo_launch_gemm_nt(P.s.dtype, 0, 0, 0, g, st);
 }
-static int conv_dgrad(const Plan& P, const void* dout, const void* wd, void* din, int Hout, int Wout, int Cout,
-                      int Hin, int Win, int Cin, bool valid, const void* relu_ref, float* colsum, DetScratch det, hipStream_t st) {
+struct PoolRoute { void* dy; unsigned char* mask; int H, W, ph, pw; };
+static GemmNT dgrad_desc(const Plan& P, const void* dout, const void* wd, void* din, int Hout, int Wout, int Cout,
+                         int Hin, int Win, int Cin, bool valid, const void* relu_ref, float* colsum, DetScratch det, const PoolRoute* rt) {
     GemmNT g; memset(&g, 0, sizeof(g));
     g.A = dout; g.Bp = wd; g.C = din;
     g.conv = 1; g.H = Hout; g.W = Wout; g.Cin = Cout;
@@ -108,7 +109,15 @@
     g.act = 0; g.alpha = 1.f; g.addend_rows = 1;
     g.relu_ref = relu_ref; g.ldr = Cin; g.colsum = colsum;
     if (P.det() && colsum) { g.colsum_part = det.p; g.colsum_part_floats = det.floats; }
+    if (rt) { g.pool_route = 1; g.pool_out = rt->dy; g.pool_mask = rt->mask; g.pool_H = rt->H; g.pool_W = rt->W; g.pool_h = rt->ph; g.pool_w = rt->pw; }
+    return g;
+}
+static int conv_dgrad(const Plan& P, const void* dout, const void* wd, void* din, int Hout, int Wout, int Cout,
+                      int Hin, int Win, int Cin, bool valid, const void* relu_ref, float* colsum, DetScratch det, hipStream_t st,
+                      const PoolRoute* rt = nullptr) {
+    const GemmNT g = dgrad_desc(P, dout, wd, din, Hout, Wout, Cout, Hin, Win, Cin, valid, relu_ref, colsum, det, rt);
     LxoTimed tm("conv_dgrad", conv_name(Cin, Cout, valid), 2.0 * P.Be * Hout * Wout * 9.0 * Cin * Cout, st);
+    if (rt) return lxo_launch_conv_igemm(g, st);
     return lxo_launch_gemm_nt(P.s.dtype, 0, 0, 0, g, st);
 }
 static int conv_wgrad(const Plan& P, const void* in, const void* dout, float* dw, int H, int W, int Cin, int Cout,
@@ -201,9 +210,12 @@
     };
     hipStream_t side = ((P.det() && !P.bf) || lxo_timer_on()) ? nullptr : g_enc_side;
     const DetScratch det_w = side ? P.det_scratch_side(ws) : det;
-    bool pending[3] = {false, false, false};
+    const int route_layers = P.unpool_layers();
+    const bool route_on = route_layers != 0;
+    int reader[3] = {0, 0, 0}, nwg = 0;
     auto acquire = [&](int i) -> int {
-        if (side && pending[i]) { HIPRC(hipStreamWaitEvent(st, g_ev_free[i], 0)); pending[i] = false; }
+        if (side && reader[i]) HIPRC(hipStreamWaitEvent(st, g_ev_free[i], 0));
+        reader[i] = 0;
         return 0;
     };
     auto wgrad = [&](const void* in, int xi, float* dw, int H, int W, int Cin, int Cout, bool valid, const void* dy_at = nullptr) -> int {
@@ -213,33 +225,80 @@
         HIPRC(hipStreamWaitEvent(side, g_ev_x, 0));
         RC(conv_wgrad(P, in, dy, dw, H, W, Cin, Cout, valid, det_w, side));
         HIPRC(hipEventRecord(g_ev_free[xi], side));
-        pending[xi] = true;
+        reader[xi] = ++nwg;
         return 0;
     };
+    auto pick = [&](int a, int b, int hint) -> int {
+        int best = -1;
+        for (int i = 0; i < 3; ++i) {
+            if (i == a || i == b) continue;
+            if (best < 0 || reader[i] < reader[best] || (reader[i] == reader[best] && i == hint)) best = i;
+        }
+        return best;
+    };
+    int cur = 0;
+    bool routed = false;
+    auto x_dest = [&](int l, int src) -> int { return route_on ? pick(src, l == first_layer ? YB[l] : -1, XB[l]) : XB[l]; };
+    auto y_dest = [&](int l, int src) -> int {
+        if (!route_on || l == first_layer) return YB[l];
+        return pick(src, (l == 4 && first_layer == 3) ? YB[3] : -1, YB[l]);
+    };
+    auto dgrad = [&](int l, const void* dy, int src, PackId wd, int Hout, int Wout, int Cout, int Hin, int Win, int Cin, bool valid,
+                     const void* relu_ref, float* colsum, const PoolRoute* below, int below_bias) -> int {
+        if (below && route_on && l - 1 >= first_layer && ((route_layers >> (l - 1)) & 1)) {
+            PoolRoute rt = *below;
+            const int di = x_dest(l - 1, src);
+            rt.dy = G[di];
+            if (lxo_conv_igemm_route_refusal(dgrad_desc(P, dy, P.pk(wp, wd), nullptr, Hout, Wout, Cout, Hin, Win, Cin, valid, nullptr, gw(below_bias), det, &rt)) == 0) {
+                RC(acquire(di));
+                RC(conv_dgrad(P, dy, P.pk(wp, wd), nullptr, Hout, Wout, Cout, Hin, Win, Cin, valid, nullptr, gw(below_bias), det, st, &rt));
+                cur = di; routed = true;
+                return 0;
+            }
+        }
+        const int di = y_dest(l, src);
+        RC(acquire(di));
+        RC(conv_dgrad(P, dy, P.pk(wp, wd), G[di], Hout, Wout, Cout, Hin, Win, Cin, valid, relu_ref, colsum, det, st));
+        cur = di; routed = false;
+        return 0;
+    };
+    auto unpool = [&](int l, WsId mask, WsId y, int bias, int H, int W, int Cc, int ph, int pw) -> int {
+        if (routed) return 0;
+        const int xi = x_dest(l, cur);
+        RC(acquire(xi));
+        if (P.pool_fused()) RC(lxo_k_maxpool_mask_bwd(P.ws<unsigned char>(ws, mask), G[cur], G[xi], gw(bias), B, H, W, Cc, ph, pw, det, st));
+        else {
+            RC(lxo_k_maxpool_relu_bwd(dt, P.ws<void>(ws, y), G[cur], G[xi], dbp(bias), B, H, W, Cc, ph, pw, st));
+            RC(dbsum(G[xi], (long long)B * H * W, Cc, bias));
+        }
+        cur = xi; routed = true;
+        return 0;
+    };
+    const PoolRoute below6 = {nullptr, P.ws<unsigned char>(ws, W_M5), P.H4, P.W2, 1, 2};
+    const PoolRoute below5 = {nullptr, P.ws<unsigned char>(ws, W_M4), P.H2, P.W2, 2, 1};
+    const PoolRoute below3 = {nullptr, P.ws<unsigned char>(ws, W_M2), P.H1, P.W1, 2, 2};
     if (P.rnn && last_layer >= 6) RC(lxo_impl_rowenc_bwd(P, prm, wp, ws, grads, st));
     for (int l = last_layer; l >= first_layer; --l) {
-        void* const X = l >= 2 ? G[XB[l]] : nullptr;
-        void* const Y = l >= 2 ? G[YB[l]] : nullptr;
-        void* const Yup = l <= 5 ? G[YB[l + 1]] : nullptr;
+        if (l == last_layer && l <= 5) { cur = YB[l + 1]; routed = false; }
         switch (l) {
         case 6:
             if (P.dimg_masked()) {
                 const void* dy6 = P.ws<void>(ws, W_DIMG);
                 RC(wgrad(P.ws<void>(ws, W_P5), XB[6], gw(P_CONV6_W), P.H6, P.W5, C, C, true, dy6));
-                RC(acquire(YB[6]));
-                RC(conv_dgrad(P, dy6, P.pk(wp, K_CONV6_D), Y, P.Hp, P.Wp, C, P.H6, P.W5, C, true, nullptr, nullptr, det, st));
+                RC(dgrad(6, dy6, -1, K_CONV6_D, P.Hp, P.Wp, C, P.H6, P.W5, C, true, nullptr, nullptr, P.cnn ? nullptr : &below6, P_CONV5_B));
                 break;
             }
             RC(acquire(XB[6]));
-            RC(lxo_k_mask_convert(dt, P.ws<float>(ws, W_DIMG), P.ws<void>(ws, W_Y6), X, dbp(P_CONV6_B), (long long)B * P.R, C, st));
-            RC(dbsum(X, (long long)B * P.R, C, P_CONV6_B));
+            RC(lxo_k_mask_convert(dt, P.ws<float>(ws, W_DIMG), P.ws<void>(ws, W_Y6), G[XB[6]], dbp(P_CONV6_B), (long long)B * P.R, C, st));
+            RC(dbsum(G[XB[6]], (long long)B * P.R, C, P_CONV6_B));
             RC(wgrad(P.ws<void>(ws, W_P5), XB[6], gw(P_CONV6_W), P.H6, P.W5, C, C, true));
-            RC(acquire(YB[6]));
-            RC(conv_dgrad(P, X, P.pk(wp, K_CONV6_D), Y, P.Hp, P.Wp, C, P.H6, P.W5, C, true, nullptr, nullptr, det, st));
+            RC(dgrad(6, G[XB[6]], XB[6], K_CONV6_D, P.Hp, P.Wp, C, P.H6, P.W5, C, true, nullptr, nullptr, P.cnn ? nullptr : &below6, P_CONV5_B));
             break;
         case 5:
-            RC(acquire(XB[5]));
             if (P.cnn) {
+                void* const Yup = G[cur];
+                void* const X = G[XB[5]];
+                RC(acquire(XB[5]));
                 const int M = B * P.H6 * P.W5;
                 if (P.det()) RC(dbsum(Yup, M, C, P_CONVS_B));
                 else RC(lxo_k_colsum_ct(dt, Yup, gw(P_CONVS_B), M, C, st));
@@ -257,44 +316,29 @@
                 RC(lxo_k_col2im_s2_relu(dt, P.ws<void>(ws, W_COLS), P.ws<void>(ws, W_Y5), X, dbp(P_CONV5_B), B, P.H4, P.W2, P.H6, P.W5, C, st));
                 RC(dbsum(X, (long long)B * P.H4 * P.W2, C, P_CONV5_B));
                 RC(wgrad(P.ws<void>(ws, W_Y4), XB[5], gw(P_CONV5_W), P.H4, P.W2, 256, C, false));
-                RC(acquire(YB[5]));
-                RC(conv_dgrad(P, X, P.pk(wp, K_CONV5_D), Y, P.H4, P.W2, C, P.H4, P.W2, 256, false, P.ws<void>(ws, W_Y4), gw(P_CONV4_B), det, st));
+                RC(dgrad(5, X, XB[5], K_CONV5_D, P.H4, P.W2, C, P.H4, P.W2, 256, false, P.ws<void>(ws, W_Y4), gw(P_CONV4_B), nullptr, 0));
                 break;
             }
-            if (P.pool_fused()) RC(lxo_k_maxpool_mask_bwd(P.ws<unsigned char>(ws, W_M5), Yup, X, gw(P_CONV5_B), B, P.H4, P.W2, C, 1, 2, det, st));
-            else RC(lxo_k_maxpool_relu_bwd(dt, P.ws<void>(ws, W_Y5), Yup, X, dbp(P_CONV5_B), B, P.H4, P.W2, C, 1, 2, st));
-            if (!P.pool_fused()) RC(dbsum(X, (long long)B * P.H4 * P.W2, C, P_CONV5_B));
-            RC(wgrad(P.ws<void>(ws, W_P4), XB[5], gw(P_CONV5_W), P.H4, P.W2, 256, C, false));
-            RC(acquire(YB[5]));
-            RC(conv_dgrad(P, X, P.pk(wp, K_CONV5_D), Y, P.H4, P.W2, C, P.H4, P.W2, 256, false, nullptr, nullptr, det, st));
+            RC(unpool(5, W_M5, W_Y5, P_CONV5_B, P.H4, P.W2, C, 1, 2));
+            RC(wgrad(P.ws<void>(ws, W_P4), cur, gw(P_CONV5_W), P.H4, P.W2, 256, C, false));
+            RC(dgrad(5, G[cur], cur, K_CONV5_D, P.H4, P.W2, C, P.H4, P.W2, 256, false, nullptr, nullptr, &below5, P_CONV4_B));
             break;
         case 4:
-            if (!P.cnn) {
-                RC(acquire(XB[4]));
-                if (P.pool_fused()) RC(lxo_k_maxpool_mask_bwd(P.ws<unsigned char>(ws, W_M4), Yup, X, gw(P_CONV4_B), B, P.H2, P.W2, 256, 2, 1, det, st));
-                else RC(lxo_k_maxpool_relu_bwd(dt, P.ws<void>(ws, W_Y4), Yup, X, dbp(P_CONV4_B), B, P.H2, P.W2, 256, 2, 1, st));
-                if (!P.pool_fused()) RC(dbsum(X, (long long)B * P.H2 * P.W2, 256, P_CONV4_B));
-            }
-            RC(wgrad(P.ws<void>(ws, W_Y3), XB[4], gw(P_CONV4_W), P.H2, P.W2, 256, 256, false));
-            RC(acquire(YB[4]));
-            RC(conv_dgrad(P, X, P.pk(wp, K_CONV4_D), Y, P.H2, P.W2, 256, P.H2, P.W2, 256, false, P.ws<void>(ws, W_Y3), gw(P_CONV3_B), det, st));
+            if (!P.cnn) RC(unpool(4, W_M4, W_Y4, P_CONV4_B, P.H2, P.W2, 256, 2, 1));
+            RC(wgrad(P.ws<void>(ws, W_Y3), cur, gw(P_CONV4_W), P.H2, P.W2, 256, 256, false));
+            RC(dgrad(4, G[cur], cur, K_CONV4_D, P.H2, P.W2, 256, P.H2, P.W2, 256, false, P.ws<void>(ws, W_Y3), gw(P_CONV3_B), nullptr, 0));
             break;
         case 3:
-            RC(wgrad(P.ws<void>(ws, W_P2), XB[3], gw(P_CONV3_W), P.H2, P.W2, 128, 256, false));
-            RC(acquire(YB[3]));
-            RC(conv_dgrad(P, X, P.pk(wp, K_CONV3_D), Y, P.H2, P.W2, 256, P.H2, P.W2, 128, false, nullptr, nullptr, det, st));
+            RC(wgrad(P.ws<void>(ws, W_P2), cur, gw(P_CONV3_W), P.H2, P.W2, 128, 256, false));
+            RC(dgrad(3, G[cur], cur, K_CONV3_D, P.H2, P.W2, 256, P.H2, P.W2, 128, false, nullptr, nullptr, &below3, P_CONV2_B));
             break;
         case 2:
-            RC(acquire(XB[2]));
-            if (P.pool_fused()) RC(lxo_k_maxpool_mask_bwd(P.ws<unsigned char>(ws, W_M2), Yup, X, gw(P_CONV2_B), B, P.H1, P.W1, 128, 2, 2, det, st));
-            else RC(lxo_k_maxpool_relu_bwd(dt, P.ws<void>(ws, W_Y2), Yup, X, dbp(P_CONV2_B), B, P.H1, P.W1, 128, 2, 2, st));
-            if (!P.pool_fused()) RC(dbsum(X, (long long)B * P.H1 * P.W1, 128, P_CONV2_B));
-            RC(wgrad(P.ws<void>(ws, W_P1), XB[2], gw(P_CONV2_W), P.H1, P.W1, 64, 128, false));
-            RC(acquire(YB[2]));
-            RC(conv_dgrad(P, X, P.pk(wp, K_CONV2_D), Y, P.H1, P.W1, 128, P.H1, P.W1, 64, false, nullptr, nullptr, det, st));
+            RC(unpool(2, W_M2, W_Y2, P_CONV2_B, P.H1, P.W1, 128, 2, 2));
+            RC(wgrad(P.ws<void>(ws, W_P1), cur, gw(P_CONV2_W), P.H1, P.W1, 64, 128, false));
+            RC(dgrad(2, G[cur], cur, K_CONV2_D, P.H1, P.W1, 128, P.H1, P.W1, 64, false, nullptr, nullptr, nullptr, 0));
             break;
         case 1:
-            RC(lxo_k_conv1_pool_bwd(dt, img, prm + P.poff[P_CONV1_W], prm + P.poff[P_CONV1_B], G[YB[2]], gw(P_CONV1_W), gw(P_CONV1_B), B, P.s.H, P.s.W, det, st));
+            RC(lxo_k_conv1_pool_bwd(dt, img, prm + P.poff[P_CONV1_W], prm + P.poff[P_CONV1_B], G[cur], gw(P_CONV1_W), gw(P_CONV1_B), B, P.s.H, P.s.W, det, st));
             break;
         default: return -4;
         }
diff --git a/latex_ocr_amd/csrc/plan.h b/latex_ocr_amd/csrc/plan.h
--- a/latex_ocr_amd/csrc/plan.h
+++ b/latex_ocr_amd/csrc/plan.h
@@ -80,6 +80,7 @@
     int attn_chunks(int nv) const;
 
     bool pool_fused() const;
+    int unpool_layers() const;
     bool dimg_masked() const { return bf && s.E % 32 == 0 && !rnn; }
     bool det() const { return !bf || s.deterministic != 0; }
     bool att_exp() const;
diff --git a/latex_ocr_amd/csrc/plan.hip b/latex_ocr_amd/csrc/plan.hip
--- a/latex_ocr_amd/csrc/plan.hip
+++ b/latex_ocr_amd/csrc/plan.hip
@@ -259,6 +259,11 @@
     if (halo < 0) { const char* b2 = getenv("LXO_CONV_2WG"); halo = (b2 && b2[0] == '0') ? 0 : 1; }
     return bf && v == 1 && halo == 1 && s.C % 128 == 0;
 }
+int Plan::unpool_layers() const {
+    static int v = -1;
+    if (v < 0) { const char* e = getenv("LXO_UNPOOL_EPI"); v = e ? atoi(e) : 1; if (v == 1) v = (1 << 5) | (1 << 2); v &= (1 << 5) | (1 << 4) | (1 << 2); }
+    return (!cnn && pool_fused()) ? v : 0;
+}
 Drop Plan::drop(int t, int row0) const {
     Drop d = {0u, 1.f, (unsigned)s.dropout_seed, t, row0, s.B};
     if (s.keep_prob > 0.f && s.keep_prob < 1.f) {
```
